# sara-nl/DDLBench

Hardware: AMD Instinct MI355X
Metric: images/sec (higher is better)
Workload: dtype bfloat16; 1 GPU; model=resnet50, global_batch=256, input=3x224x224, parallelism=dp1

## Files before the change

ddlbench_amd/ops/conv.py:

```python

from __future__ import annotations

import os

import torch
import torch.nn as nn
import torch.nn.functional as F

from ddlbench_amd import ops as _ops

_WGRAD = os.environ.get("DDLB_WGRAD", "mfma")

_CL = torch.channels_last


def _dw_to_weight_layout(dw32, weight):
    K, C, R, S = weight.shape
    return dw32.view(K, R, S, C).permute(0, 3, 1, 2).to(weight.dtype)


def _conv_backward(ctx, dy, add=None):
    ext = _ops.require_extension()
    x, weight = ctx.saved_tensors
    dy = dy.contiguous(memory_format=_CL)
    dx = dw = None
    if ctx.needs_input_grad[0]:
        w_perm = weight.permute(1, 2, 3, 0).contiguous()
        dx = ext.conv_igemm_dgrad(dy, w_perm, x.size(0), x.size(1),
                                  x.size(2), x.size(3), ctx.stride,
                                  ctx.pad, add)
    if ctx.needs_input_grad[1]:
        if _WGRAD == "mfma":
            dw = _dw_to_weight_layout(
                ext.conv_igemm_wgrad(x, dy, weight.shape[2],
                                     weight.shape[3], ctx.stride,
                                     ctx.pad), weight)
        else:
            dw = torch.ops.aten.convolution_backward(
                dy, x, weight, None, [ctx.stride, ctx.stride],
                [ctx.pad, ctx.pad], [1, 1], False, [0, 0], 1,
                [False, True, False])[1]
    return dx, dw


class _ConvMFMA(torch.autograd.Function):
    @staticmethod
    def forward(ctx, x, weight, stride, pad):
        ext = _ops.require_extension()
        x = x.contiguous(memory_format=_CL)
        w = weight.contiguous(memory_format=_CL)
        y = ext.conv_igemm_fwd(x, w, stride, pad)
        ctx.save_for_backward(x, weight)
        ctx.stride = stride
        ctx.pad = pad
        return y

    @staticmethod
    def backward(ctx, dy):
        dx, dw = _conv_backward(ctx, dy)
        return dx, dw, None, None


def conv2d_mfma(x, weight, stride=1, pad=0):
    return _ConvMFMA.apply(x, weight, stride, pad)


class _ConvMFMAJoin(torch.autograd.Function):

    @staticmethod
    def forward(ctx, x, weight, stride, pad):
        ext = _ops.require_extension()
        w = weight.contiguous(memory_format=_CL)
        y = ext.conv_igemm_fwd(x, w, stride, pad)
        ctx.save_for_backward(x, weight)
        ctx.stride = stride
        ctx.pad = pad
        ctx.set_materialize_grads(False)
        return y, x

    @staticmethod
    def backward(ctx, dy, dskip):
        if dy is None:
            return dskip, None, None, None
        if dskip is not None:
            dskip = dskip.contiguous(memory_format=_CL)
        dx, dw = _conv_backward(ctx, dy, dskip)
        return dx, dw, None, None


def join_enabled() -> bool:
    return os.environ.get("DDLB_JOIN", "1") != "0"


def mfma_eligible(conv: nn.Conv2d, x_dtype=torch.bfloat16) -> bool:
    return (x_dtype == torch.bfloat16
            and conv.groups == 1
            and conv.dilation == (1, 1)
            and conv.bias is None
            and conv.in_channels % 8 == 0
            and conv.out_channels % 8 == 0
            and conv.stride[0] == conv.stride[1]
            and conv.padding[0] == conv.padding[1]
            and conv.kernel_size[0] == conv.kernel_size[1])


class _NativeConv2d(nn.Module):

    tag = ""

    def __init__(self, conv: nn.Conv2d):
        super().__init__()
        self.in_channels = conv.in_channels
        self.out_channels = conv.out_channels
        self.kernel_size = conv.kernel_size
        self.stride = conv.stride[0]
        self.padding = conv.padding[0]
        self.weight = conv.weight

    def native(self, x):
        raise NotImplementedError

    def forward(self, x):
        if x.is_cuda and x.dtype == torch.bfloat16:
            return self.native(x)
        return F.conv2d(x, self.weight, None, self.stride, self.padding)

    def extra_repr(self):
        return (f"{self.in_channels}, {self.out_channels}, "
                f"k={self.kernel_size}, stride={self.stride}, "
                f"pad={self.padding} [{self.tag}]")


class Conv2dMFMA(_NativeConv2d):

    tag = "mfma"

    def native(self, x):
        return conv2d_mfma(x, self.weight, self.stride, self.padding)

    def forward_join(self, x):
        if (x.is_cuda and x.dtype == torch.bfloat16 and x.dim() == 4
                and x.is_contiguous(memory_format=_CL) and join_enabled()):
            return _ConvMFMAJoin.apply(x, self.weight, self.stride,
                                       self.padding)
        return self.forward(x), x


class _ConvStem(torch.autograd.Function):

    @staticmethod
    def forward(ctx, x, weight, stride, pad):
        ext = _ops.require_extension()
        x = x.contiguous(memory_format=_CL)
        w = weight.contiguous(memory_format=_CL)
        y = ext.conv_stem_fwd(x, w, stride, pad)
        ctx.save_for_backward(x, weight)
        ctx.stride = stride
        ctx.pad = pad
        return y

    @staticmethod
    def backward(ctx, dy):
        ext = _ops.require_extension()
        x, weight = ctx.saved_tensors
        dy = dy.contiguous(memory_format=_CL)
        dx = dw = None
        if ctx.needs_input_grad[0]:
            dx = torch.ops.aten.convolution_backward(
                dy, x, weight, None, [ctx.stride, ctx.stride],
                [ctx.pad, ctx.pad], [1, 1], False, [0, 0], 1,
                [True, False, False])[0]
        if ctx.needs_input_grad[1]:
            dw = _dw_to_weight_layout(
                ext.conv_stem_wgrad(x, dy, weight.shape[2], weight.shape[3],
                                    ctx.stride, ctx.pad), weight)
        return dx, dw, None, None


def conv2d_stem(x, weight, stride=1, pad=0):
    return _ConvStem.apply(x, weight, stride, pad)


def stem_eligible(conv: nn.Conv2d, x_dtype=torch.bfloat16) -> bool:
    return (x_dtype == torch.bfloat16
            and conv.groups == 1
            and conv.dilation == (1, 1)
            and conv.bias is None
            and 1 <= conv.in_channels <= 4
            and conv.out_channels % 8 == 0
            and 8 <= conv.out_channels <= 128
            and conv.kernel_size[0] == conv.kernel_size[1]
            and conv.kernel_size[0] in (3, 5, 7)
            and conv.stride[0] == conv.stride[1]
            and conv.stride[0] in (1, 2)
            and not isinstance(conv.padding, str)
            and conv.padding[0] == conv.padding[1]
            and 0 <= conv.padding[0] <= conv.kernel_size[0] // 2)


class Conv2dStem(_NativeConv2d):

    tag = "stem"

    def native(self, x):
        return conv2d_stem(x, self.weight, self.stride, self.padding)


def convert_convs(model: nn.Module, dtype=torch.bfloat16,
                  stem=None) -> int:
    if stem is None:
        stem = os.environ.get("DDLB_STEM", "library")
    if stem not in ("native", "library"):
        raise ValueError(f"stem must be 'native' or 'library', got {stem!r}")
    count = 0
    for parent in model.modules():
        for name, child in list(parent.named_children()):
            if not isinstance(child, nn.Conv2d):
                continue
            if mfma_eligible(child, dtype):
                setattr(parent, name, Conv2dMFMA(child))
                count += 1
            elif stem == "native" and stem_eligible(child, dtype):
                setattr(parent, name, Conv2dStem(child))
                count += 1
    if dtype == torch.bfloat16 and \
            os.environ.get("DDLB_MAXPOOL", "1") != "0":
        from ddlbench_amd.ops.pool import convert_maxpools
        count += convert_maxpools(model)
    return count
```

ddlbench_amd/ops/csrc/bindings.hip:

```cpp

#include <torch/extension.h>
#include <c10/hip/HIPStream.h>
#include <hip/hip_runtime.h>
#include <hip/hip_bf16.h>

#include <algorithm>
#include <stdexcept>
#include <unordered_map>
#include <vector>

#include "launchers.h"

using namespace ddlb;

namespace {

hipStream_t cur_stream() {
  return c10::hip::getCurrentHIPStream().stream();
}

void check_gpu_contig(const torch::Tensor& t, const char* name) {
  TORCH_CHECK(t.is_cuda(), name, " must be on the HIP device");
  TORCH_CHECK(t.is_contiguous(), name, " must be contiguous");
}

bool is_bf16(const torch::Tensor& t) {
  return t.scalar_type() == at::kBFloat16;
}

template <typename T>
T* dptr(const torch::Tensor& t) {
  return reinterpret_cast<T*>(t.data_ptr());
}

template <typename F>
auto dispatch_f32_bf16(bool bf16, F&& fn) {
  return bf16 ? fn(__hip_bfloat16{}) : fn(float{});
}
template <typename F>
auto dispatch_f32_bf16(const torch::Tensor& x, F&& fn) {
  return dispatch_f32_bf16(is_bf16(x), fn);
}

using WsCache = std::unordered_map<int, torch::Tensor>;
torch::Tensor cached_ws(WsCache& cache, const torch::Tensor& like,
                        at::ScalarType dtype, int64_t min_numel,
                        int64_t grow_floor = 0, bool zeroed = false) {
  torch::Tensor& t = cache[(int)like.get_device()];
  if (!t.defined() || t.numel() < min_numel) {
    const int64_t cap = std::max(min_numel, grow_floor);
    const auto opt = like.options().dtype(dtype);
    t = zeroed ? torch::zeros({cap}, opt) : torch::empty({cap}, opt);
  }
  return t;
}

torch::Tensor zero_page(const torch::Tensor& like) {
  static WsCache zp;
  return cached_ws(zp, like, at::kBFloat16, 16, 0, true);
}

torch::Tensor bn_sums_workspace(const torch::Tensor& like, int64_t C,
                                int64_t S) {
  static WsCache ws;
  return cached_ws(ws, like, at::kDouble, 2 * C * S, 1 << 18);
}

void check_conv_operand(const torch::Tensor& t, const char* name,
                        const char* op = "conv_igemm") {
  TORCH_CHECK(t.is_cuda() && t.scalar_type() == at::kBFloat16, op,
              ": bf16 HIP tensors only");
  TORCH_CHECK(t.is_contiguous(at::MemoryFormat::ChannelsLast), name,
              " must be channels_last");
}

int conv_out_size(int64_t H, int64_t pad, int64_t R, int64_t stride) {
  return (int)((H + 2 * pad - R) / stride + 1);
}

void check_conv_geometry(const char* op, int64_t N, int64_t H, int64_t W,
                         int64_t R, int64_t S, int64_t stride,
                         int64_t pad) {
  TORCH_CHECK(stride >= 1, op, ": stride must be >= 1");
  TORCH_CHECK(pad >= 0, op, ": pad must be >= 0");
  TORCH_CHECK(R >= 1 && S >= 1, op, ": kernel dims must be >= 1");
  TORCH_CHECK(N >= 1 && H >= 1 && W >= 1, op, ": empty input");
  TORCH_CHECK(H + 2 * pad >= R && W + 2 * pad >= S, op,
              ": kernel larger than the padded input");
}

void check_conv_dy(const char* op, const torch::Tensor& dy, int64_t N,
                   int64_t H, int64_t W, int64_t R, int64_t S,
                   int64_t stride, int64_t pad) {
  TORCH_CHECK(dy.size(0) == N, op, ": dy batch does not match x");
  TORCH_CHECK(dy.size(2) == conv_out_size(H, pad, R, stride) &&
                  dy.size(3) == conv_out_size(W, pad, S, stride),
              op, ": dy spatial dims do not match (H,W,R,S,stride,pad)");
}

torch::Tensor empty_nhwc(const torch::Tensor& like, int64_t N, int64_t C,
                         int64_t H, int64_t W) {
  return torch::empty({N, C, H, W}, like.options().memory_format(
                                        at::MemoryFormat::ChannelsLast));
}

}

void fused_sgd(torch::Tensor ptr_params, torch::Tensor ptr_grads,
               torch::Tensor ptr_moms, torch::Tensor prefix, int64_t total,
               double lr, double momentum, double weight_decay,
               bool first_step, bool bf16) {
  check_gpu_contig(ptr_params, "ptr_params");
  dispatch_f32_bf16(bf16, [&](auto tag) {
    launch_fused_sgd<decltype(tag)>(
        dptr<uintptr_t>(ptr_params), dptr<uintptr_t>(ptr_grads),
        dptr<uintptr_t>(ptr_moms), dptr<int64_t>(prefix),
        (int)ptr_params.numel(), total, (float)lr, (float)momentum,
        (float)weight_decay, first_step, cur_stream());
  });
}

void fused_adam(torch::Tensor ptr_params, torch::Tensor ptr_grads,
                torch::Tensor ptr_ms, torch::Tensor ptr_vs,
                torch::Tensor prefix, int64_t total, double lr,
                double beta1, double beta2, double eps,
                double weight_decay, double bc1, double bc2,
                bool decoupled_wd, bool bf16) {
  check_gpu_contig(ptr_params, "ptr_params");
  dispatch_f32_bf16(bf16, [&](auto tag) {
    launch_fused_adam<decltype(tag)>(
        dptr<uintptr_t>(ptr_params), dptr<uintptr_t>(ptr_grads),
        dptr<uintptr_t>(ptr_ms), dptr<uintptr_t>(ptr_vs),
        dptr<int64_t>(prefix), (int)ptr_params.numel(), total, (float)lr,
        (float)beta1, (float)beta2, (float)eps, (float)weight_decay,
        (float)bc1, (float)bc2, decoupled_wd, cur_stream());
  });
}

std::vector<torch::Tensor> bn_act_fwd(
    torch::Tensor x, c10::optional<torch::Tensor> res, torch::Tensor gamma,
    torch::Tensor beta, c10::optional<torch::Tensor> running_mean,
    c10::optional<torch::Tensor> running_var, bool training, double momentum,
    double eps, int64_t act, bool nhwc) {
  TORCH_CHECK(x.is_cuda(), "x must be on the HIP device");
  TORCH_CHECK(x.dim() == 4, "x must be 4-D");
  TORCH_CHECK(nhwc ? x.is_contiguous(at::MemoryFormat::ChannelsLast)
                   : x.is_contiguous(), "x layout mismatch");
  const int64_t N = x.size(0), C = x.size(1), HW = x.size(2) * x.size(3);
  auto s = cur_stream();
  auto fopt = x.options().dtype(at::kFloat);
  torch::Tensor mean = torch::empty({C}, fopt);
  torch::Tensor invstd = torch::empty({C}, fopt);
  if (training) {
    const int64_t S =
        bn_reduce_gridS(N, C, HW, nhwc, (int)x.element_size());
    torch::Tensor sums = bn_sums_workspace(x, C, S);
    dispatch_f32_bf16(x, [&](auto tag) {
      using T = decltype(tag);
      launch_bn_stats<T>(dptr<T>(x), dptr<double>(sums), N, C, HW, S, nhwc,
                         s);
    });
    launch_bn_finalize(
        dptr<double>(sums), dptr<float>(mean), dptr<float>(invstd),
        running_mean ? dptr<float>(*running_mean) : nullptr,
        running_var ? dptr<float>(*running_var) : nullptr, C, S,
        (double)(N * HW), (float)eps, (float)momentum, s);
  } else {
    TORCH_CHECK(running_mean && running_var,
                "eval mode needs running stats");
    mean.copy_(*running_mean);
    invstd.copy_((running_var->to(at::kFloat) + eps).rsqrt());
  }
  torch::Tensor y = torch::empty_like(x);
  const int64_t total = x.numel();
  torch::Tensor msk;
  const bool want_mask =
      training && act != 0 && nhwc && is_bf16(x) && C % 8 == 0;
  if (want_mask)
    msk = torch::empty({total / 8}, x.options().dtype(at::kByte));
  const bool mask_written = dispatch_f32_bf16(x, [&](auto tag) {
    using T = decltype(tag);
    return launch_bn_apply<T>(
        dptr<T>(x), res ? dptr<T>(*res) : nullptr, dptr<T>(y),
        dptr<float>(mean), dptr<float>(invstd), dptr<float>(gamma),
        dptr<float>(beta),
        want_mask ? msk.data_ptr<unsigned char>() : nullptr,
        C, HW, total, (int)act, nhwc, s);
  });
  if (mask_written) return {y, mean, invstd, msk};
  return {y, mean, invstd};
}

std::vector<torch::Tensor> bn_act_bwd(torch::Tensor dy,
                                      c10::optional<torch::Tensor> y_opt,
                                      torch::Tensor x, torch::Tensor mean,
                                      torch::Tensor invstd,
                                      torch::Tensor gamma, int64_t act,
                                      bool training, bool need_dres,
                                      bool nhwc,
                                      c10::optional<torch::Tensor> msk) {
  TORCH_CHECK(dy.is_cuda(), "dy must be on the HIP device");
  TORCH_CHECK(y_opt || msk,
              "bn_act_bwd needs y or the 1-bit activation mask");
  const int64_t N = x.size(0), C = x.size(1), HW = x.size(2) * x.size(3);
  auto s = cur_stream();
  auto fopt = x.options().dtype(at::kFloat);
  const int64_t S = bn_reduce_gridS(N, C, HW, nhwc, (int)x.element_size());
  torch::Tensor sums = bn_sums_workspace(x, C, S);
  torch::Tensor dgamma = torch::empty({C}, fopt);
  torch::Tensor dbeta = torch::empty({C}, fopt);
  torch::Tensor k = torch::empty({3, C}, fopt);
  torch::Tensor dx = torch::empty_like(x);
  torch::Tensor dres =
      need_dres ? torch::empty_like(x) : torch::Tensor();
  const int64_t total = x.numel();
  const unsigned char* mp =
      msk ? msk->data_ptr<unsigned char>() : nullptr;
  if (!is_bf16(x)) {
    TORCH_CHECK(y_opt, "fp32 backward needs y");
    mp = nullptr;
  }
  dispatch_f32_bf16(x, [&](auto tag) {
    using T = decltype(tag);
    const T* yp = y_opt ? dptr<T>(*y_opt) : nullptr;
    launch_bn_bwd_reduce<T>(dptr<T>(dy), yp, dptr<T>(x), dptr<float>(mean),
                            dptr<float>(invstd), dptr<double>(sums), mp, N,
                            C, HW, S, (int)act, nhwc, s);
    launch_bn_bwd_finalize(dptr<double>(sums), dptr<float>(gamma),
                           dptr<float>(invstd), dptr<float>(dgamma),
                           dptr<float>(dbeta), dptr<float>(k), C, S,
                           (double)(N * HW), training, s);
    launch_bn_bwd_dx<T>(dptr<T>(dy), yp, dptr<T>(x), dptr<float>(mean),
                        dptr<float>(invstd), dptr<float>(k), dptr<T>(dx),
                        need_dres ? dptr<T>(dres) : nullptr, mp, C, HW,
                        total, (int)act, nhwc, s);
  });
  if (need_dres) return {dx, dgamma, dbeta, dres};
  return {dx, dgamma, dbeta};
}

std::vector<torch::Tensor> ce_fwd(torch::Tensor logits,
                                  torch::Tensor target) {
  check_gpu_contig(logits, "logits");
  const int64_t B = logits.size(0), K = logits.size(1);
  auto s = cur_stream();
  auto fopt = logits.options().dtype(at::kFloat);
  torch::Tensor lse = torch::empty({B}, fopt);
  torch::Tensor loss_sum = torch::zeros({1}, fopt);
  dispatch_f32_bf16(logits, [&](auto tag) {
    using T = decltype(tag);
    launch_ce_fwd<T>(dptr<T>(logits), dptr<int64_t>(target),
                     dptr<float>(lse), dptr<float>(loss_sum), B, K, s);
  });
  return {loss_sum, lse};
}

torch::Tensor ce_bwd(torch::Tensor logits, torch::Tensor target,
                     torch::Tensor lse, torch::Tensor gscale) {
  const int64_t B = logits.size(0), K = logits.size(1);
  auto s = cur_stream();
  torch::Tensor dx = torch::empty_like(logits);
  dispatch_f32_bf16(logits, [&](auto tag) {
    using T = decltype(tag);
    launch_ce_bwd<T>(dptr<T>(logits), dptr<int64_t>(target),
                     dptr<float>(lse), dptr<float>(gscale), dptr<T>(dx), B,
                     K, s);
  });
  return dx;
}

torch::Tensor conv_igemm_fwd(torch::Tensor x, torch::Tensor w,
                             int64_t stride, int64_t pad) {
  TORCH_CHECK(x.dim() == 4 && w.dim() == 4, "conv_igemm: 4-D tensors only");
  check_conv_operand(x, "x", "conv_igemm");
  check_conv_operand(w, "w", "conv_igemm");
  TORCH_CHECK(w.device() == x.device(), "conv_igemm: w must be on x's device");
  const int N = x.size(0), C = x.size(1), H = x.size(2), W = x.size(3);
  const int K = w.size(0), R = w.size(2), S = w.size(3);
  TORCH_CHECK(w.size(1) == C, "conv_igemm: weight C does not match x");
  TORCH_CHECK(C % 8 == 0, "conv_igemm fwd needs C % 8 == 0");
  TORCH_CHECK(K >= 1, "conv_igemm: empty weight");
  check_conv_geometry("conv_igemm", N, H, W, R, S, stride, pad);
  const int OH = conv_out_size(H, pad, R, stride);
  const int OW = conv_out_size(W, pad, S, stride);
  auto y = empty_nhwc(x, N, K, OH, OW);
  launch_conv_igemm(x.data_ptr(), w.data_ptr(), y.data_ptr(),
                    zero_page(x).data_ptr(), N, H, W, C, K, OH, OW, R, S,
                    (int)stride, (int)pad, 0, nullptr,
                    cur_stream());
  return y;
}

torch::Tensor conv_igemm_dgrad(torch::Tensor dy, torch::Tensor w_perm,
                               int64_t N, int64_t C, int64_t H, int64_t W,
                               int64_t stride, int64_t pad,
                               c10::optional<torch::Tensor> add) {
  TORCH_CHECK(dy.dim() == 4 && w_perm.dim() == 4,
              "conv_igemm: 4-D tensors only");
  check_conv_operand(dy, "dy", "conv_igemm");
  TORCH_CHECK(w_perm.is_cuda() && w_perm.scalar_type() == at::kBFloat16 &&
                  w_perm.device() == dy.device(),
              "conv_igemm: w_perm must be a bf16 tensor on dy's device");
  TORCH_CHECK(w_perm.is_contiguous(), "w_perm must be contiguous");
  if (add) {
    check_conv_operand(*add, "add", "conv_igemm");
    TORCH_CHECK(add->dim() == 4 && add->size(0) == N &&
                    add->size(1) == C && add->size(2) == H &&
                    add->size(3) == W,
                "add must have dx's shape (N,C,H,W)");
    TORCH_CHECK(add->device() == dy.device(),
                "add must be on dy's device");
  }
  const int K = dy.size(1), OH = dy.size(2), OW = dy.size(3);
  const int R = w_perm.size(1), S = w_perm.size(2);
  TORCH_CHECK(K % 8 == 0, "conv_igemm dgrad needs K % 8 == 0");
  TORCH_CHECK(C >= 1 && w_perm.size(0) == C && w_perm.size(3) == K,
              "conv_igemm: w_perm must be (C,R,S,K) for dx's C and dy's K");
  check_conv_geometry("conv_igemm", N, H, W, R, S, stride, pad);
  check_conv_dy("conv_igemm", dy, N, H, W, R, S, stride, pad);
  auto dx = empty_nhwc(dy, N, C, H, W);
  const bool sparse = stride == 2 && (R == 1 || S == 1);
  if (sparse) dx.zero_();
  launch_conv_igemm(dy.data_ptr(), w_perm.data_ptr(), dx.data_ptr(),
                    zero_page(dy).data_ptr(), (int)N, (int)H, (int)W,
                    (int)C, K, OH, OW, R, S, (int)stride, (int)pad,
                    1, add && !sparse ? add->data_ptr() : nullptr,
                    cur_stream());
  if (add && sparse) dx.add_(*add);
  return dx;
}

torch::Tensor conv_igemm_wgrad(torch::Tensor x, torch::Tensor dy,
                               int64_t R, int64_t S, int64_t stride,
                               int64_t pad) {
  TORCH_CHECK(x.dim() == 4 && dy.dim() == 4, "conv_wgrad: 4-D tensors only");
  check_conv_operand(x, "x", "conv_wgrad");
  check_conv_operand(dy, "dy", "conv_wgrad");
  TORCH_CHECK(dy.device() == x.device(),
              "conv_wgrad: dy must be on x's device");
  const int N = x.size(0), C = x.size(1), H = x.size(2), W = x.size(3);
  const int K = dy.size(1), OH = dy.size(2), OW = dy.size(3);
  TORCH_CHECK(C % 8 == 0 && K % 8 == 0,
              "conv_wgrad needs C %% 8 == 0 and K %% 8 == 0");
  TORCH_CHECK(K >= 1, "conv_wgrad: empty dy");
  check_conv_geometry("conv_wgrad", N, H, W, R, S, stride, pad);
  check_conv_dy("conv_wgrad", dy, N, H, W, R, S, stride, pad);
  auto dw = torch::empty({K, R * S * C},
                         x.options().dtype(at::kFloat));
  static WsCache wgws;
  auto part = cached_ws(wgws, x, at::kFloat, kConvWgradPartCap);
  launch_conv_wgrad(x.data_ptr(), dy.data_ptr(), dw.data_ptr<float>(),
                    part.data_ptr<float>(), (long)part.numel(),
                    zero_page(x).data_ptr(), N, H, W, C, K, OH, OW, (int)R,
                    (int)S, (int)stride, (int)pad, cur_stream());
  return dw;
}

py::list conv_igemm_plan_py(int64_t N, int64_t C, int64_t H, int64_t W,
                            int64_t K, int64_t R, int64_t S, int64_t stride,
                            int64_t pad, bool dgrad) {
  check_conv_geometry("conv_igemm_plan", N, H, W, R, S, stride, pad);
  const ConvIgemmPlan plan = conv_igemm_plan(
      (int)N, (int)H, (int)W, (int)C, (int)K,
      conv_out_size(H, pad, R, stride), conv_out_size(W, pad, S, stride),
      (int)R, (int)S, (int)stride, (int)pad, dgrad ? 1 : 0);
  py::list out;
  for (int i = 0; i < plan.n; ++i) {
    const ConvIgemmLaunch& e = plan.e[i];
    py::dict d;
    d["structure"] = e.v2 ? "v2" : "v1";
    d["mode"] = e.mode;
    d["BM"] = e.bm;
    d["BN"] = e.bn;
    d["LIN"] = e.lin != 0;
    d["M"] = e.M;
    d["Nd"] = e.Nd;
    d["Kd"] = e.Kd;
    d["cls"] = py::make_tuple(e.cls_a, e.cls_b);
    d["taps"] = py::make_tuple(e.nr, e.ns);
    out.append(d);
  }
  return out;
}

py::dict conv_wgrad_plan_py(int64_t N, int64_t C, int64_t H, int64_t W,
                            int64_t K, int64_t R, int64_t S, int64_t stride,
                            int64_t pad) {
  check_conv_geometry("conv_wgrad_plan", N, H, W, R, S, stride, pad);
  const ConvWgradPlan pl = conv_wgrad_plan(
      (int)N, (int)C, (int)K, conv_out_size(H, pad, R, stride),
      conv_out_size(W, pad, S, stride), (int)R, (int)S, (int)stride,
      (int)pad, kConvWgradPartCap);
  py::dict d;
  d["TK"] = pl.tk;
  d["TR"] = pl.tr;
  d["ring"] = pl.ring;
  d["r1"] = pl.r1 != 0;
  d["split"] = pl.split;
  d["p_per"] = pl.p_per;
  d["steps"] = pl.steps;
  d["tail"] = pl.tail;
  d["psb"] = pl.psb;
  return d;
}

static void check_stem_shape(int64_t C, int64_t K, int64_t R, int64_t S,
                             int64_t stride, int64_t pad) {
  TORCH_CHECK(C >= 1 && C <= 4, "conv_stem needs 1 <= C <= 4");
  TORCH_CHECK(R == S && (R == 3 || R == 5 || R == 7),
              "conv_stem needs a square 3x3, 5x5 or 7x7 kernel");
  TORCH_CHECK(stride == 1 || stride == 2, "conv_stem needs stride 1 or 2");
  TORCH_CHECK(pad >= 0 && pad <= R / 2, "conv_stem needs 0 <= pad <= R/2");
  TORCH_CHECK(K % 8 == 0 && K >= 8 && K <= 128,
              "conv_stem needs K % 8 == 0 and K <= 128");
}

torch::Tensor conv_stem_fwd(torch::Tensor x, torch::Tensor w,
                            int64_t stride, int64_t pad) {
  TORCH_CHECK(x.dim() == 4 && w.dim() == 4, "conv_stem: 4-D tensors only");
  check_conv_operand(x, "x", "conv_stem");
  check_conv_operand(w, "w", "conv_stem");
  const int N = x.size(0), C = x.size(1), H = x.size(2), W = x.size(3);
  const int K = w.size(0), R = w.size(2), S = w.size(3);
  TORCH_CHECK(w.size(1) == C, "conv_stem: weight C mismatch");
  check_stem_shape(C, K, R, S, stride, pad);
  const int OH = conv_out_size(H, pad, R, stride);
  const int OW = conv_out_size(W, pad, S, stride);
  TORCH_CHECK(N >= 1 && H + 2 * pad >= R && W + 2 * pad >= S,
              "conv_stem: empty output");
  auto y = empty_nhwc(x, N, K, OH, OW);
  launch_conv_stem_fwd(x.data_ptr(), w.data_ptr(), y.data_ptr(), N, H, W, C,
                       K, OH, OW, R, (int)stride, (int)pad, cur_stream());
  return y;
}

torch::Tensor conv_stem_wgrad(torch::Tensor x, torch::Tensor dy, int64_t R,
                              int64_t S, int64_t stride, int64_t pad) {
  TORCH_CHECK(x.dim() == 4 && dy.dim() == 4, "conv_stem: 4-D tensors only");
  check_conv_operand(x, "x", "conv_stem");
  check_conv_operand(dy, "dy", "conv_stem");
  const int N = x.size(0), C = x.size(1), H = x.size(2), W = x.size(3);
  const int K = dy.size(1), OH = dy.size(2), OW = dy.size(3);
  check_stem_shape(C, K, R, S, stride, pad);
  TORCH_CHECK(N >= 1 && dy.size(0) == N && OH >= 1 && OW >= 1 &&
                  OH == conv_out_size(H, pad, R, stride) &&
                  OW == conv_out_size(W, pad, S, stride),
              "conv_stem: dy shape does not match x");
  const int64_t total = (int64_t)K * R * S * C;
  auto dw = torch::empty({K, R * S * C}, x.options().dtype(at::kFloat));
  static WsCache stws;
  auto part = cached_ws(stws, x, at::kFloat,
                        total * conv_stem_wgrad_chunks(N, OH, OW, K));
  launch_conv_stem_wgrad(x.data_ptr(), dy.data_ptr(), dw.data_ptr<float>(),
                         part.data_ptr<float>(), N, H, W, C, K, OH, OW,
                         (int)R, (int)stride, (int)pad, cur_stream());
  return dw;
}

std::vector<torch::Tensor> maxpool_fwd(torch::Tensor x, int64_t k,
                                       int64_t stride, int64_t pad) {
  TORCH_CHECK(x.is_cuda() && x.scalar_type() == at::kBFloat16,
              "maxpool: bf16 HIP tensors only");
  TORCH_CHECK(x.is_contiguous(at::MemoryFormat::ChannelsLast),
              "maxpool: x must be channels_last");
  const int64_t N = x.size(0), C = x.size(1);
  const int H = (int)x.size(2), W = (int)x.size(3);
  TORCH_CHECK(C % 8 == 0, "maxpool needs C %% 8 == 0");
  const int OH = (H + 2 * (int)pad - (int)k) / (int)stride + 1;
  const int OW = (W + 2 * (int)pad - (int)k) / (int)stride + 1;
  auto y = torch::empty({N, C, OH, OW},
                        x.options().memory_format(
                            at::MemoryFormat::ChannelsLast));
  auto idx = torch::empty({N * OH * OW * C},
                          x.options().dtype(at::kByte));
  launch_maxpool_fwd(x.data_ptr(), y.data_ptr(),
                     idx.data_ptr<unsigned char>(), N, C, H, W, OH, OW,
                     (int)k, (int)stride, (int)pad, cur_stream());
  return {y, idx};
}

torch::Tensor maxpool_bwd(torch::Tensor dy, torch::Tensor idx,
                          int64_t H, int64_t W, int64_t k,
                          int64_t stride, int64_t pad) {
  TORCH_CHECK(dy.is_cuda() && dy.scalar_type() == at::kBFloat16,
              "maxpool: bf16 HIP tensors only");
  TORCH_CHECK(dy.is_contiguous(at::MemoryFormat::ChannelsLast),
              "maxpool: dy must be channels_last");
  const int64_t N = dy.size(0), C = dy.size(1);
  const int OH = (int)dy.size(2), OW = (int)dy.size(3);
  auto dx = torch::empty({N, C, H, W},
                         dy.options().memory_format(
                             at::MemoryFormat::ChannelsLast));
  launch_maxpool_bwd(dy.data_ptr(), idx.data_ptr<unsigned char>(),
                     dx.data_ptr(), N, C, (int)H, (int)W, OH, OW,
                     (int)k, (int)stride, (int)pad, cur_stream());
  return dx;
}

torch::Tensor dw3x3_fwd(torch::Tensor x, torch::Tensor w, int64_t stride,
                        bool nhwc) {
  TORCH_CHECK(x.is_cuda(), "x must be on the HIP device");
  check_gpu_contig(w, "w");
  const int64_t N = x.size(0), C = x.size(1), H = x.size(2), W = x.size(3);
  const int64_t OH = (H + 2 - 3) / stride + 1, OW = (W + 2 - 3) / stride + 1;
  auto s = cur_stream();
  torch::Tensor y = nhwc
      ? torch::empty({N, C, OH, OW}, x.options().memory_format(
            at::MemoryFormat::ChannelsLast))
      : torch::empty({N, C, OH, OW}, x.options());
  dispatch_f32_bf16(x, [&](auto tag) {
    using T = decltype(tag);
    launch_dw3x3_fwd<T>(dptr<T>(x), dptr<float>(w), dptr<T>(y), N, C, H, W,
                        OH, OW, (int)stride, nhwc, s);
  });
  return y;
}

std::vector<torch::Tensor> dw3x3_bwd(torch::Tensor x, torch::Tensor w,
                                     torch::Tensor dy, int64_t stride,
                                     bool need_dx, bool need_dw,
                                     bool nhwc) {
  const int64_t N = x.size(0), C = x.size(1), H = x.size(2), W = x.size(3);
  const int64_t OH = dy.size(2), OW = dy.size(3);
  auto s = cur_stream();
  torch::Tensor dx, dwt;
  if (need_dx) {
    dx = torch::empty_like(x);
    dispatch_f32_bf16(x, [&](auto tag) {
      using T = decltype(tag);
      launch_dw3x3_bwd_dx<T>(dptr<T>(dy), dptr<float>(w), dptr<T>(dx), N, C,
                             H, W, OH, OW, (int)stride, nhwc, s);
    });
  }
  if (need_dw) {
    torch::Tensor acc = torch::zeros({C * 9}, x.options().dtype(at::kDouble));
    dispatch_f32_bf16(x, [&](auto tag) {
      using T = decltype(tag);
      launch_dw3x3_bwd_dw<T>(dptr<T>(x), dptr<T>(dy), dptr<double>(acc), N,
                             C, H, W, OH, OW, (int)stride, nhwc, s);
    });
    dwt = acc.to(at::kFloat).view({C, 1, 3, 3});
  }
  return {dx, dwt};
}

torch::Tensor revert_varlen(torch::Tensor x, torch::Tensor lengths) {
  check_gpu_contig(x, "x");
  TORCH_CHECK(x.dim() == 3, "x must be (T, B, F)");
  TORCH_CHECK(lengths.scalar_type() == at::kLong, "lengths must be int64");
  const int64_t T = x.size(0), B = x.size(1), F = x.size(2);
  auto out = torch::empty_like(x);
  auto s = cur_stream();
  dispatch_f32_bf16(x, [&](auto tag) {
    using E = decltype(tag);
    launch_revert_varlen<E>(dptr<E>(x), dptr<E>(out),
                            dptr<int64_t>(lengths), T, B, F, s);
  });
  return out;
}

torch::Tensor varlen_mask(torch::Tensor lengths, int64_t T) {
  TORCH_CHECK(lengths.is_cuda(), "lengths must be on the HIP device");
  const int64_t B = lengths.size(0);
  auto mask = torch::empty({T, B}, lengths.options().dtype(at::kByte));
  launch_varlen_mask(dptr<int64_t>(lengths), dptr<uint8_t>(mask), T, B,
                     cur_stream());
  return mask;
}

PYBIND11_MODULE(TORCH_EXTENSION_NAME, m) {
  m.doc() = "ddlbench_amd gfx950 HIP kernels";
  m.def("fused_sgd", &fused_sgd, "fused multi-tensor SGD step");
  m.def("fused_adam", &fused_adam, "fused multi-tensor Adam/AdamW step");
  m.def("bn_act_fwd", &bn_act_fwd, "fused BN+act(+res) forward");
  m.def("set_bn_variant", &set_bn_variant,
        "BN kernel variant for A/B probes (0 auto, 1 scalar-group, 2 vec)");
  m.def("bn_act_bwd", &bn_act_bwd, "fused BN+act(+res) backward");
  m.def("maxpool_fwd", &maxpool_fwd, "NHWC bf16 max-pool forward");
  m.def("maxpool_bwd", &maxpool_bwd, "NHWC bf16 max-pool backward");
  m.def("conv_igemm_fwd", &conv_igemm_fwd,
        "NHWC bf16 MFMA implicit-GEMM conv forward");
  m.def("conv_igemm_dgrad", &conv_igemm_dgrad,
        "NHWC bf16 MFMA implicit-GEMM conv data-grad (+ optional addend)",
        py::arg("dy"), py::arg("w_perm"), py::arg("N"), py::arg("C"),
        py::arg("H"), py::arg("W"), py::arg("stride"), py::arg("pad"),
        py::arg("add") = py::none());
  m.def("conv_igemm_wgrad", &conv_igemm_wgrad,
        "NHWC bf16 MFMA implicit-GEMM conv weight-grad (fp32 out)");
  m.def("conv_igemm_plan", &conv_igemm_plan_py,
        "launches conv_igemm_fwd/dgrad make for a shape (host only)",
        py::arg("N"), py::arg("C"), py::arg("H"), py::arg("W"),
        py::arg("K"), py::arg("R"), py::arg("S"), py::arg("stride"),
        py::arg("pad"), py::arg("dgrad"));
  m.def("conv_wgrad_plan", &conv_wgrad_plan_py,
        "tile/split/steps conv_igemm_wgrad uses for a shape (host only)",
        py::arg("N"), py::arg("C"), py::arg("H"), py::arg("W"),
        py::arg("K"), py::arg("R"), py::arg("S"), py::arg("stride"),
        py::arg("pad"));
  m.def("conv_stem_fwd", &conv_stem_fwd,
        "NHWC bf16 MFMA stem conv (C < 8) forward");
  m.def("conv_stem_wgrad", &conv_stem_wgrad,
        "NHWC bf16 MFMA stem conv (C < 8) weight-grad (fp32 out)");
  m.def("ce_fwd", &ce_fwd, "cross-entropy forward");
  m.def("ce_bwd", &ce_bwd, "cross-entropy backward");
  m.def("revert_varlen", &revert_varlen,
        "reverse each batch element's valid time prefix (T,B,F)");
  m.def("varlen_mask", &varlen_mask, "valid-timestep mask (T,B) uint8");
  m.def("dw3x3_fwd", &dw3x3_fwd, "depthwise 3x3 forward");
  m.def("dw3x3_bwd", &dw3x3_bwd, "depthwise 3x3 backward");
}
```

ddlbench_amd/ops/csrc/bn_act.hip:

```cpp

#include "common.h"
#include "launchers.h"
#include <stdint.h>
#include <stdexcept>
#include <string>

namespace {

template <int ACT> DEV float act_fwd(float v) {
  if (ACT == 1) return fmaxf(v, 0.f);
  if (ACT == 2) return fminf(fmaxf(v, 0.f), 6.f);
  return v;
}

template <int ACT> DEV float act_mask(float y) {
  if (ACT == 1) return y > 0.f ? 1.f : 0.f;
  if (ACT == 2) return (y > 0.f && y < 6.f) ? 1.f : 0.f;
  return 1.f;
}

}

int g_bn_variant = 0;
void ddlb::set_bn_variant(int v) { g_bn_variant = v; }

template <typename T>
__global__ void bn_stats_kernel(const T* __restrict__ x, double* __restrict__ sums,
                                int64_t N, int64_t C, int64_t HW) {
  __shared__ double tmp[8];
  const int64_t c = blockIdx.x;
  const int64_t total = N * HW;
  const int64_t per = (total + gridDim.y - 1) / gridDim.y;
  const int64_t begin = (int64_t)blockIdx.y * per;
  const int64_t end = i64min(begin + per, total);
  double s = 0.0, ss = 0.0;
  for (int64_t i = begin + threadIdx.x; i < end; i += blockDim.x) {
    const int64_t n = i / HW, r = i - n * HW;
    const float v = to_f32(x[(n * C + c) * HW + r]);
    s += v;
    ss += fma((double)v, (double)v, 0.0);
  }
  auto op = [](double v) { return wave_reduce_sum(v); };
  s = block_reduce(s, tmp, op, 0.0);
  __syncthreads();
  ss = block_reduce(ss, tmp, op, 0.0);
  if (threadIdx.x == 0) {
    sums[((int64_t)blockIdx.y * 2 + 0) * C + c] = s;
    sums[((int64_t)blockIdx.y * 2 + 1) * C + c] = ss;
  }
}

template <typename T>
__global__ void bn_stats_nhwc_kernel(const T* __restrict__ x,
                                     double* __restrict__ sums,
                                     int64_t rows, int64_t C, int CG) {
  __shared__ double tmp[2 * 256];
  const int ci = threadIdx.x % CG;
  const int rj = threadIdx.x / CG;
  const int RG = blockDim.x / CG;
  const int64_t c = (int64_t)blockIdx.x * CG + ci;
  const bool active = (c < C) && (rj < RG);
  const int64_t per = (rows + gridDim.y - 1) / gridDim.y;
  const int64_t begin = (int64_t)blockIdx.y * per;
  const int64_t end = i64min(begin + per, rows);
  double s = 0.0, ss = 0.0;
  if (active) {
    int64_t r = begin + rj;
    const int64_t step = RG;
    for (; r + 3 * step < end; r += 4 * step) {
      float v0 = to_f32(x[(r + 0 * step) * C + c]);
      float v1 = to_f32(x[(r + 1 * step) * C + c]);
      float v2 = to_f32(x[(r + 2 * step) * C + c]);
      float v3 = to_f32(x[(r + 3 * step) * C + c]);
      s += (double)v0 + v1 + v2 + v3;
      ss += fma((double)v0, v0, fma((double)v1, v1,
                fma((double)v2, v2, (double)v3 * v3)));
    }
    for (; r < end; r += step) {
      const float v = to_f32(x[r * C + c]);
      s += v;
      ss += fma((double)v, (double)v, 0.0);
    }
  }
  tmp[threadIdx.x] = s;
  tmp[256 + threadIdx.x] = ss;
  __syncthreads();
  if (rj == 0 && c < C) {
    for (int j = 1; j < RG; ++j) {
      s += tmp[j * CG + ci];
      ss += tmp[256 + j * CG + ci];
    }
    sums[((int64_t)blockIdx.y * 2 + 0) * C + c] = s;
    sums[((int64_t)blockIdx.y * 2 + 1) * C + c] = ss;
  }
}

template <typename T>
__global__ void bn_stats_nhwc_vec_kernel(const T* __restrict__ x,
                                         double* __restrict__ sums,
                                         int64_t rows, int64_t C, int CG8) {
  typedef __attribute__((ext_vector_type(8))) short short8x;
  __shared__ float tmp[2][256][8];
  const int ci = threadIdx.x % CG8;
  const int rj = threadIdx.x / CG8;
  const int RG = blockDim.x / CG8;
  const int64_t c0 = ((int64_t)blockIdx.x * CG8 + ci) * 8;
  const bool active = (c0 < C) && (rj < RG);
  const int64_t per = (rows + gridDim.y - 1) / gridDim.y;
  const int64_t begin = (int64_t)blockIdx.y * per;
  const int64_t end = i64min(begin + per, rows);
  float s[8] = {0, 0, 0, 0, 0, 0, 0, 0};
  float ss[8] = {0, 0, 0, 0, 0, 0, 0, 0};
  if (active) {
    const short8x* xv = reinterpret_cast<const short8x*>(x);
    for (int64_t r = begin + rj; r < end; r += RG) {
      short8x v = xv[(r * C + c0) / 8];
#pragma unroll
      for (int j = 0; j < 8; ++j) {
        __hip_bfloat16 h;
        unsigned short u = (unsigned short)v[j];
        __builtin_memcpy(&h, &u, 2);
        const float f = __bfloat162float(h);
        s[j] += f;
        ss[j] = fmaf(f, f, ss[j]);
      }
    }
  }
#pragma unroll
  for (int j = 0; j < 8; ++j) {
    tmp[0][threadIdx.x][j] = s[j];
    tmp[1][threadIdx.x][j] = ss[j];
  }
  __syncthreads();
  if (rj == 0 && c0 < C) {
    for (int g = 1; g < RG; ++g)
#pragma unroll
      for (int j = 0; j < 8; ++j) {
        s[j] += tmp[0][g * CG8 + ci][j];
        ss[j] += tmp[1][g * CG8 + ci][j];
      }
#pragma unroll
    for (int j = 0; j < 8; ++j) {
      sums[((int64_t)blockIdx.y * 2 + 0) * C + c0 + j] = (double)s[j];
      sums[((int64_t)blockIdx.y * 2 + 1) * C + c0 + j] = (double)ss[j];
    }
  }
}

__global__ void bn_stats_nhwc_vec_f32_kernel(const float* __restrict__ x,
                                             double* __restrict__ sums,
                                             int64_t rows, int64_t C,
                                             int CG4) {
  typedef __attribute__((ext_vector_type(4))) float float4x;
  __shared__ float tmp[2][256][4];
  const int ci = threadIdx.x % CG4;
  const int rj = threadIdx.x / CG4;
  const int RG = blockDim.x / CG4;
  const int64_t c0 = ((int64_t)blockIdx.x * CG4 + ci) * 4;
  const bool active = (c0 < C) && (rj < RG);
  const int64_t per = (rows + gridDim.y - 1) / gridDim.y;
  const int64_t begin = (int64_t)blockIdx.y * per;
  const int64_t end = i64min(begin + per, rows);
  float s[4] = {0, 0, 0, 0}, ss[4] = {0, 0, 0, 0};
  if (active) {
    const float4x* xv = reinterpret_cast<const float4x*>(x);
    for (int64_t r = begin + rj; r < end; r += RG) {
      float4x v = xv[(r * C + c0) / 4];
#pragma unroll
      for (int j = 0; j < 4; ++j) {
        s[j] += v[j];
        ss[j] = fmaf(v[j], v[j], ss[j]);
      }
    }
  }
#pragma unroll
  for (int j = 0; j < 4; ++j) {
    tmp[0][threadIdx.x][j] = s[j];
    tmp[1][threadIdx.x][j] = ss[j];
  }
  __syncthreads();
  if (rj == 0 && c0 < C) {
    for (int g = 1; g < RG; ++g)
#pragma unroll
      for (int j = 0; j < 4; ++j) {
        s[j] += tmp[0][g * CG4 + ci][j];
        ss[j] += tmp[1][g * CG4 + ci][j];
      }
#pragma unroll
    for (int j = 0; j < 4; ++j) {
      sums[((int64_t)blockIdx.y * 2 + 0) * C + c0 + j] = (double)s[j];
      sums[((int64_t)blockIdx.y * 2 + 1) * C + c0 + j] = (double)ss[j];
    }
  }
}

__global__ void bn_finalize_kernel(const double* __restrict__ sums,
                                   float* __restrict__ mean,
                                   float* __restrict__ invstd,
                                   float* __restrict__ running_mean,
                                   float* __restrict__ running_var,
                                   int64_t C, int64_t S, double count,
                                   float eps, float momentum) {
  __shared__ double tmp[16];
  const int64_t c = blockIdx.x;
  double s = 0.0, ss = 0.0;
  for (int64_t b = threadIdx.x; b < S; b += blockDim.x) {
    s += sums[(b * 2 + 0) * C + c];
    ss += sums[(b * 2 + 1) * C + c];
  }
  auto op = [](double v) { return wave_reduce_sum(v); };
  s = block_reduce(s, tmp, op, 0.0);
  __syncthreads();
  ss = block_reduce(ss, tmp, op, 0.0);
  if (threadIdx.x != 0) return;
  const double m = s / count;
  double var = ss / count - m * m;
  var = var < 0.0 ? 0.0 : var;
  mean[c] = (float)m;
  invstd[c] = (float)rsqrt(var + (double)eps);
  if (running_mean != nullptr) {
    const double unbiased = count > 1.0 ? var * count / (count - 1.0) : var;
    running_mean[c] = (1.f - momentum) * running_mean[c] + momentum * (float)m;
    running_var[c] = (1.f - momentum) * running_var[c] + momentum * (float)unbiased;
  }
}

template <typename T, int ACT, bool ADD>
__global__ void bn_apply_kernel(const T* __restrict__ x,
                                const T* __restrict__ res,
                                T* __restrict__ y,
                                const float* __restrict__ mean,
                                const float* __restrict__ invstd,
                                const float* __restrict__ gamma,
                                const float* __restrict__ beta,
                                int64_t C, int64_t cdiv, int64_t total) {
  const int64_t stride = (int64_t)gridDim.x * blockDim.x;
  for (int64_t i = (int64_t)blockIdx.x * blockDim.x + threadIdx.x; i < total;
       i += stride) {
    const int64_t c = (i / cdiv) % C;
    float v = (to_f32(x[i]) - mean[c]) * invstd[c] * gamma[c] + beta[c];
    if (ADD) v += to_f32(res[i]);
    y[i] = from_f32<T>(act_fwd<ACT>(v));
  }
}

typedef __attribute__((ext_vector_type(8))) short short8v;
typedef __attribute__((ext_vector_type(4))) float float4v;

template <typename T> struct vec8;
template <> struct vec8<float> {
  using type = __attribute__((ext_vector_type(8))) float;
};
template <> struct vec8<__hip_bfloat16> { using type = short8v; };

DEV float elt_f32(const short8v& v, int j) {
  __hip_bfloat16 h;
  unsigned short u = (unsigned short)v[j];
  __builtin_memcpy(&h, &u, 2);
  return __bfloat162float(h);
}
DEV float elt_f32(const __attribute__((ext_vector_type(8))) float& v,
                  int j) { return v[j]; }

template <typename T>
DEV void set_elt(short8v& v, int j, float f) {
  __hip_bfloat16 h = __float2bfloat16(f);
  unsigned short u;
  __builtin_memcpy(&u, &h, 2);
  v[j] = (short)u;
}
template <typename T>
DEV void set_elt(__attribute__((ext_vector_type(8))) float& v, int j,
                 float f) { v[j] = f; }

template <typename T, int ACT, bool ADD, bool NHWC>
__global__ void bn_apply_vec_kernel(const T* __restrict__ x,
                                    const T* __restrict__ res,
                                    T* __restrict__ y,
                                    const float* __restrict__ mean,
                                    const float* __restrict__ invstd,
                                    const float* __restrict__ gamma,
                                    const float* __restrict__ beta,
                                    int64_t C, int64_t cdiv,
                                    int64_t total8) {
  using V = typename vec8<T>::type;
  const V* xv = reinterpret_cast<const V*>(x);
  const V* rv = reinterpret_cast<const V*>(res);
  V* yv = reinterpret_cast<V*>(y);
  const int64_t stride = (int64_t)gridDim.x * blockDim.x;
  for (int64_t i = (int64_t)blockIdx.x * blockDim.x + threadIdx.x;
       i < total8; i += stride) {
    const int64_t e0 = i * 8;
    V vx = xv[i];
    V vr;
    if (ADD) vr = rv[i];
    V vy;
    if (NHWC) {
      const int64_t c0 = e0 % C;
#pragma unroll
      for (int j = 0; j < 8; ++j) {
        const int64_t c = c0 + j;
        float v = (elt_f32(vx, j) - mean[c]) * invstd[c] * gamma[c]
                  + beta[c];
        if (ADD) v += elt_f32(vr, j);
        set_elt<T>(vy, j, act_fwd<ACT>(v));
      }
    } else {
      const int64_t c = (e0 / cdiv) % C;
      const float mu = mean[c], is = invstd[c], g = gamma[c], b = beta[c];
#pragma unroll
      for (int j = 0; j < 8; ++j) {
        float v = (elt_f32(vx, j) - mu) * is * g + b;
        if (ADD) v += elt_f32(vr, j);
        set_elt<T>(vy, j, act_fwd<ACT>(v));
      }
    }
    yv[i] = vy;
  }
}

template <typename T, int ACT, bool ADD, bool NHWC>
__global__ void bn_bwd_dx_vec_kernel(const T* __restrict__ dy,
                                     const T* __restrict__ y,
                                     const T* __restrict__ x,
                                     const float* __restrict__ mean,
                                     const float* __restrict__ invstd,
                                     const float* __restrict__ k,
                                     T* __restrict__ dx,
                                     T* __restrict__ dres, int64_t C,
                                     int64_t cdiv, int64_t total8) {
  using V = typename vec8<T>::type;
  const V* dyv = reinterpret_cast<const V*>(dy);
  const V* yv = reinterpret_cast<const V*>(y);
  const V* xv = reinterpret_cast<const V*>(x);
  V* dxv = reinterpret_cast<V*>(dx);
  V* drv = reinterpret_cast<V*>(dres);
  const int64_t stride = (int64_t)gridDim.x * blockDim.x;
  for (int64_t i = (int64_t)blockIdx.x * blockDim.x + threadIdx.x;
       i < total8; i += stride) {
    const int64_t e0 = i * 8;
    V vdy = dyv[i], vy = yv[i], vx = xv[i];
    V vdx, vdr;
#pragma unroll
    for (int j = 0; j < 8; ++j) {
      const int64_t c = NHWC ? (e0 % C + j) : ((e0 / cdiv) % C);
      const float g = elt_f32(vdy, j) * act_mask<ACT>(elt_f32(vy, j));
      const float xhat = (elt_f32(vx, j) - mean[c]) * invstd[c];
      set_elt<T>(vdx, j, k[c] * (g - k[C + c] - xhat * k[2 * C + c]));
      if (ADD) set_elt<T>(vdr, j, g);
    }
    dxv[i] = vdx;
    if (ADD) drv[i] = vdr;
  }
}

template <typename T, int ACT, bool ADD>
__global__ void bn_apply_nhwc_kernel2(const T* __restrict__ x,
                                      const T* __restrict__ res,
                                      T* __restrict__ y,
                                      const float* __restrict__ mean,
                                      const float* __restrict__ invstd,
                                      const float* __restrict__ gamma,
                                      const float* __restrict__ beta,
                                      unsigned char* __restrict__ msk,
                                      int64_t rows, int64_t C, int CG8) {
  typedef __attribute__((ext_vector_type(8))) short short8x;
  const int ci = threadIdx.x % CG8;
  const int rj = threadIdx.x / CG8;
  const int RG = blockDim.x / CG8;
  const int64_t c0 = ((int64_t)blockIdx.x * CG8 + ci) * 8;
  if (c0 >= C || rj >= RG) return;
  float sc[8], sh[8];
#pragma unroll
  for (int j = 0; j < 8; ++j) {
    sc[j] = invstd[c0 + j] * gamma[c0 + j];
    sh[j] = beta[c0 + j] - mean[c0 + j] * sc[j];
  }
  const int64_t per = (rows + gridDim.y - 1) / gridDim.y;
  const int64_t begin = (int64_t)blockIdx.y * per;
  const int64_t end = i64min(begin + per, rows);
  const short8x* xv = reinterpret_cast<const short8x*>(x);
  const short8x* rv = reinterpret_cast<const short8x*>(res);
  short8x* yv = reinterpret_cast<short8x*>(y);
  for (int64_t r = begin + rj; r < end; r += RG) {
    const int64_t i8 = (r * C + c0) / 8;
    short8x vx = xv[i8];
    short8x vr;
    if (ADD) vr = rv[i8];
    short8x vy;
    unsigned mbits = 0;
#pragma unroll
    for (int j = 0; j < 8; ++j) {
      __hip_bfloat16 h;
      unsigned short u = (unsigned short)vx[j];
      __builtin_memcpy(&h, &u, 2);
      float v = fmaf(__bfloat162float(h), sc[j], sh[j]);
      if (ADD) {
        u = (unsigned short)vr[j];
        __builtin_memcpy(&h, &u, 2);
        v += __bfloat162float(h);
      }
      if (ACT != 0 && act_mask<ACT>(v) > 0.f) mbits |= 1u << j;
      h = __float2bfloat16(act_fwd<ACT>(v));
      __builtin_memcpy(&u, &h, 2);
      vy[j] = (short)u;
    }
    yv[i8] = vy;
    if (ACT != 0 && msk != nullptr) msk[i8] = (unsigned char)mbits;
  }
}

template <typename T, int ACT, bool ADD, bool MASKED = false>
__global__ void bn_bwd_dx_nhwc_kernel2(const T* __restrict__ dy,
                                       const T* __restrict__ y,
                                       const T* __restrict__ x,
                                       const float* __restrict__ mean,
                                       const float* __restrict__ invstd,
                                       const float* __restrict__ k,
                                       T* __restrict__ dx,
                                       T* __restrict__ dres,
                                       const unsigned char* __restrict__ msk,
                                       int64_t rows,
                                       int64_t C, int CG8) {
  typedef __attribute__((ext_vector_type(8))) short short8x;
  const int ci = threadIdx.x % CG8;
  const int rj = threadIdx.x / CG8;
  const int RG = blockDim.x / CG8;
  const int64_t c0 = ((int64_t)blockIdx.x * CG8 + ci) * 8;
  if (c0 >= C || rj >= RG) return;
  float k1[8], k2[8], k3[8], mu[8], is[8];
#pragma unroll
  for (int j = 0; j < 8; ++j) {
    k1[j] = k[c0 + j];
    k2[j] = k[C + c0 + j];
    k3[j] = k[2 * C + c0 + j];
    mu[j] = mean[c0 + j];
    is[j] = invstd[c0 + j];
  }
  const int64_t per = (rows + gridDim.y - 1) / gridDim.y;
  const int64_t begin = (int64_t)blockIdx.y * per;
  const int64_t end = i64min(begin + per, rows);
  const short8x* dyv = reinterpret_cast<const short8x*>(dy);
  const short8x* yv = reinterpret_cast<const short8x*>(y);
  const short8x* xv = reinterpret_cast<const short8x*>(x);
  short8x* dxv = reinterpret_cast<short8x*>(dx);
  short8x* drv = reinterpret_cast<short8x*>(dres);
  for (int64_t r = begin + rj; r < end; r += RG) {
    const int64_t i8 = (r * C + c0) / 8;
    short8x vdy = dyv[i8], vx = xv[i8];
    short8x vy;
    unsigned mb = 0;
    if (MASKED) mb = msk[i8];
    else vy = yv[i8];
    short8x vdx, vdr;
#pragma unroll
    for (int j = 0; j < 8; ++j) {
      __hip_bfloat16 h;
      unsigned short u;
      u = (unsigned short)vdy[j];
      __builtin_memcpy(&h, &u, 2);
      const float fdy = __bfloat162float(h);
      float gate;
      if (MASKED) {
        gate = (float)((mb >> j) & 1u);
      } else {
        u = (unsigned short)vy[j];
        __builtin_memcpy(&h, &u, 2);
        gate = act_mask<ACT>(__bfloat162float(h));
      }
      u = (unsigned short)vx[j];
      __builtin_memcpy(&h, &u, 2);
      const float fx = __bfloat162float(h);
      const float g = fdy * gate;
      const float xhat = (fx - mu[j]) * is[j];
      h = __float2bfloat16(k1[j] * (g - k2[j] - xhat * k3[j]));
      __builtin_memcpy(&u, &h, 2);
      vdx[j] = (short)u;
      if (ADD) {
        h = __float2bfloat16(g);
        __builtin_memcpy(&u, &h, 2);
        vdr[j] = (short)u;
      }
    }
    dxv[i8] = vdx;
    if (ADD) drv[i8] = vdr;
  }
}

template <typename T, int ACT>
__global__ void bn_bwd_reduce_kernel(const T* __restrict__ dy,
                                     const T* __restrict__ y,
                                     const T* __restrict__ x,
                                     const float* __restrict__ mean,
                                     const float* __restrict__ invstd,
                                     double* __restrict__ sums,
                                     int64_t N, int64_t C, int64_t HW) {
  __shared__ double tmp[8];
  const int64_t c = blockIdx.x;
  const float mu = mean[c], is = invstd[c];
  const int64_t total = N * HW;
  const int64_t per = (total + gridDim.y - 1) / gridDim.y;
  const int64_t begin = (int64_t)blockIdx.y * per;
  const int64_t end = i64min(begin + per, total);
  double sdy = 0.0, sdyx = 0.0;
  for (int64_t i = begin + threadIdx.x; i < end; i += blockDim.x) {
    const int64_t n = i / HW, r = i - n * HW;
    const int64_t idx = (n * C + c) * HW + r;
    const float g = to_f32(dy[idx]) * act_mask<ACT>(to_f32(y[idx]));
    const float xhat = (to_f32(x[idx]) - mu) * is;
    sdy += g;
    sdyx += fma((double)g, (double)xhat, 0.0);
  }
  auto op = [](double v) { return wave_reduce_sum(v); };
  sdy = block_reduce(sdy, tmp, op, 0.0);
  __syncthreads();
  sdyx = block_reduce(sdyx, tmp, op, 0.0);
  if (threadIdx.x == 0) {
    sums[((int64_t)blockIdx.y * 2 + 0) * C + c] = sdy;
    sums[((int64_t)blockIdx.y * 2 + 1) * C + c] = sdyx;
  }
}

template <typename T, int ACT, bool MASKED = false>
__global__ void bn_bwd_reduce_nhwc_kernel(const T* __restrict__ dy,
                                          const T* __restrict__ y,
                                          const T* __restrict__ x,
                                          const float* __restrict__ mean,
                                          const float* __restrict__ invstd,
                                          double* __restrict__ sums,
                                          const unsigned char* __restrict__
                                              msk,
                                          int64_t rows, int64_t C, int CG) {
  __shared__ double tmp[2 * 256];
  const int ci = threadIdx.x % CG;
  const int rj = threadIdx.x / CG;
  const int RG = blockDim.x / CG;
  const int64_t c = (int64_t)blockIdx.x * CG + ci;
  const bool active = (c < C) && (rj < RG);
  const int64_t per = (rows + gridDim.y - 1) / gridDim.y;
  const int64_t begin = (int64_t)blockIdx.y * per;
  const int64_t end = i64min(begin + per, rows);
  double sdy = 0.0, sdyx = 0.0;
  if (active) {
    const float mu = mean[c], is = invstd[c];
    const int cbit = (int)(c & 7);
    for (int64_t r = begin + rj; r < end; r += RG) {
      const int64_t idx = r * C + c;
      float gate;
      if (MASKED)
        gate = (float)((msk[idx >> 3] >> cbit) & 1u);
      else
        gate = act_mask<ACT>(to_f32(y[idx]));
      const float g = to_f32(dy[idx]) * gate;
      const float xhat = (to_f32(x[idx]) - mu) * is;
      sdy += g;
      sdyx += fma((double)g, (double)xhat, 0.0);
    }
  }
  tmp[threadIdx.x] = sdy;
  tmp[256 + threadIdx.x] = sdyx;
  __syncthreads();
  if (rj == 0 && c < C) {
    for (int j = 1; j < RG; ++j) {
      sdy += tmp[j * CG + ci];
      sdyx += tmp[256 + j * CG + ci];
    }
    sums[((int64_t)blockIdx.y * 2 + 0) * C + c] = sdy;
    sums[((int64_t)blockIdx.y * 2 + 1) * C + c] = sdyx;
  }
}

template <typename T, int ACT, bool MASKED = false>
__global__ void bn_bwd_reduce_nhwc_vec_kernel(
    const T* __restrict__ dy, const T* __restrict__ y,
    const T* __restrict__ x, const float* __restrict__ mean,
    const float* __restrict__ invstd, double* __restrict__ sums,
    const unsigned char* __restrict__ msk,
    int64_t rows, int64_t C, int CG8) {
  typedef __attribute__((ext_vector_type(8))) short short8x;
  __shared__ float tmp[2][256][8];
  const int ci = threadIdx.x % CG8;
  const int rj = threadIdx.x / CG8;
  const int RG = blockDim.x / CG8;
  const int64_t c0 = ((int64_t)blockIdx.x * CG8 + ci) * 8;
  const bool active = (c0 < C) && (rj < RG);
  const int64_t per = (rows + gridDim.y - 1) / gridDim.y;
  const int64_t begin = (int64_t)blockIdx.y * per;
  const int64_t end = i64min(begin + per, rows);
  float sdy[8] = {0, 0, 0, 0, 0, 0, 0, 0};
  float sdyx[8] = {0, 0, 0, 0, 0, 0, 0, 0};
  float mu[8], is[8];
  if (active) {
#pragma unroll
    for (int j = 0; j < 8; ++j) {
      mu[j] = mean[c0 + j];
      is[j] = invstd[c0 + j];
    }
    const short8x* dyv = reinterpret_cast<const short8x*>(dy);
    const short8x* yv = reinterpret_cast<const short8x*>(y);
    const short8x* xv = reinterpret_cast<const short8x*>(x);
    for (int64_t r = begin + rj; r < end; r += RG) {
      const int64_t i8 = (r * C + c0) / 8;
      short8x vdy = dyv[i8], vx = xv[i8];
      short8x vy;
      unsigned mb = 0;
      if (MASKED) mb = msk[i8];
      else vy = yv[i8];
#pragma unroll
      for (int j = 0; j < 8; ++j) {
        __hip_bfloat16 h;
        unsigned short u;
        u = (unsigned short)vdy[j];
        __builtin_memcpy(&h, &u, 2);
        const float fdy = __bfloat162float(h);
        float gate;
        if (MASKED) {
          gate = (float)((mb >> j) & 1u);
        } else {
          u = (unsigned short)vy[j];
          __builtin_memcpy(&h, &u, 2);
          gate = act_mask<ACT>(__bfloat162float(h));
        }
        u = (unsigned short)vx[j];
        __builtin_memcpy(&h, &u, 2);
        const float fx = __bfloat162float(h);
        const float g = fdy * gate;
        sdy[j] += g;
        sdyx[j] = fmaf(g, (fx - mu[j]) * is[j], sdyx[j]);
      }
    }
  }
#pragma unroll
  for (int j = 0; j < 8; ++j) {
    tmp[0][threadIdx.x][j] = sdy[j];
    tmp[1][threadIdx.x][j] = sdyx[j];
  }
  __syncthreads();
  if (rj == 0 && c0 < C) {
    for (int g = 1; g < RG; ++g)
#pragma unroll
      for (int j = 0; j < 8; ++j) {
        sdy[j] += tmp[0][g * CG8 + ci][j];
        sdyx[j] += tmp[1][g * CG8 + ci][j];
      }
#pragma unroll
    for (int j = 0; j < 8; ++j) {
      sums[((int64_t)blockIdx.y * 2 + 0) * C + c0 + j] = (double)sdy[j];
      sums[((int64_t)blockIdx.y * 2 + 1) * C + c0 + j] = (double)sdyx[j];
    }
  }
}

__global__ void bn_bwd_finalize_kernel(const double* __restrict__ sums,
                                       const float* __restrict__ gamma,
                                       const float* __restrict__ invstd,
                                       float* __restrict__ dgamma,
                                       float* __restrict__ dbeta,
                                       float* __restrict__ k,
                                       int64_t C, int64_t S, double count,
                                       int training) {
  __shared__ double tmp[16];
  const int64_t c = blockIdx.x;
  double sdy = 0.0, sdyx = 0.0;
  for (int64_t b = threadIdx.x; b < S; b += blockDim.x) {
    sdy += sums[(b * 2 + 0) * C + c];
    sdyx += sums[(b * 2 + 1) * C + c];
  }
  auto op = [](double v) { return wave_reduce_sum(v); };
  sdy = block_reduce(sdy, tmp, op, 0.0);
  __syncthreads();
  sdyx = block_reduce(sdyx, tmp, op, 0.0);
  if (threadIdx.x != 0) return;
  dgamma[c] = (float)sdyx;
  dbeta[c] = (float)sdy;
  k[c] = gamma[c] * invstd[c];
  k[C + c] = training ? (float)(sdy / count) : 0.f;
  k[2 * C + c] = training ? (float)(sdyx / count) : 0.f;
}

template <typename T, int ACT, bool ADD>
__global__ void bn_bwd_dx_kernel(const T* __restrict__ dy,
                                 const T* __restrict__ y,
                                 const T* __restrict__ x,
                                 const float* __restrict__ mean,
                                 const float* __restrict__ invstd,
                                 const float* __restrict__ k,
                                 T* __restrict__ dx, T* __restrict__ dres,
                                 int64_t C, int64_t cdiv, int64_t total) {
  const int64_t stride = (int64_t)gridDim.x * blockDim.x;
  for (int64_t i = (int64_t)blockIdx.x * blockDim.x + threadIdx.x; i < total;
       i += stride) {
    const int64_t c = (i / cdiv) % C;
    const float g = to_f32(dy[i]) * act_mask<ACT>(to_f32(y[i]));
    const float xhat = (to_f32(x[i]) - mean[c]) * invstd[c];
    dx[i] = from_f32<T>(k[c] * (g - k[C + c] - xhat * k[2 * C + c]));
    if (ADD) dres[i] = from_f32<T>(g);
  }
}

static inline int elementwise_grid(int64_t total, int block) {
  int64_t want = (total + block - 1) / block;
  return (int)i64min(want > 0 ? want : 1, 256 * 8);
}


struct BnGeom { bool vec; int64_t cblocks, S; };

static BnGeom bn_reduce_geom(int64_t rows, int64_t C, int elsize) {
  BnGeom g;
  const bool vec_ok = (elsize == 2 && C % 8 == 0) ||
                      (elsize == 4 && C % 4 == 0);
  g.vec = vec_ok && (g_bn_variant == 2 ||
                     (g_bn_variant == 0 && C <= 512 && elsize == 2));
  if (g.vec) {
    const int64_t lanes = elsize == 2 ? C / 8 : C / 4;
    const int64_t CG = i64min(lanes, 64);
    g.cblocks = (lanes + CG - 1) / CG;
  } else {
    const int64_t CG = C >= 64 ? 64 : C;
    g.cblocks = (C + CG - 1) / CG;
  }
  g.S = i64min(i64max(rows / 16, 1), i64max(2048 / g.cblocks, 1));
  return g;
}

int64_t ddlb::bn_reduce_gridS(int64_t N, int64_t C, int64_t HW, int nhwc,
                              int elsize) {
  if (nhwc) return bn_reduce_geom(N * HW, C, elsize).S;
  int64_t S = i64min((N * HW + 255) / 256, i64max(2048 / C, 1));
  return i64max(S, 1);
}

template <typename T>
void ddlb::launch_bn_stats(const T* x, double* sums, int64_t N, int64_t C,
                           int64_t HW, int64_t S, int nhwc,
                           hipStream_t stream) {
  const int block = 256;
  if (nhwc) {
    const int64_t rows = N * HW;
    const BnGeom g = bn_reduce_geom(rows, C, (int)sizeof(T));
    if (g.vec && sizeof(T) == 2) {
      const int CG8 = (int)i64min(C / 8, 64);
      hipLaunchKernelGGL((bn_stats_nhwc_vec_kernel<T>),
                         dim3(g.cblocks, S),
                         dim3(block), 0, stream, x, sums, rows, C, CG8);
    } else if (g.vec && sizeof(T) == 4) {
      const int CG4 = (int)i64min(C / 4, 64);
      hipLaunchKernelGGL(bn_stats_nhwc_vec_f32_kernel, dim3(g.cblocks, S),
                         dim3(block), 0, stream, (const float*)x, sums,
                         rows, C, CG4);
    } else {
      const int CG = C >= 64 ? 64 : (int)C;
      hipLaunchKernelGGL((bn_stats_nhwc_kernel<T>), dim3(g.cblocks, S),
                         dim3(block), 0, stream, x, sums, rows, C, CG);
    }
  } else {
    hipLaunchKernelGGL((bn_stats_kernel<T>), dim3(C, S), dim3(block), 0,
                       stream, x, sums, N, C, HW);
  }
  HIP_CHECK_LAST();
}

void ddlb::launch_bn_finalize(double* sums, float* mean, float* invstd,
                              float* rm, float* rv, int64_t C, int64_t S,
                              double count, float eps, float momentum,
                              hipStream_t stream) {
  const int block = 1024;
  hipLaunchKernelGGL(bn_finalize_kernel, dim3((unsigned)C),
                     dim3(block), 0, stream, sums, mean, invstd, rm, rv, C,
                     S, count, eps, momentum);
  HIP_CHECK_LAST();
}

template <typename T>
bool ddlb::launch_bn_apply(const T* x, const T* res, T* y, const float* mean,
                           const float* invstd, const float* gamma,
                           const float* beta, unsigned char* msk, int64_t C,
                           int64_t HW, int64_t total, int act, int nhwc,
                           hipStream_t stream) {
  const int block = 256;
  const int64_t cdiv = nhwc ? 1 : HW;
  const bool vec8ok = (total % 8 == 0) &&
                      (nhwc ? (C % 8 == 0) : (HW % 8 == 0));
  const int64_t rows_nhwc = nhwc ? total / C : 0;
  if (nhwc && sizeof(T) == 2 && C % 8 == 0 && g_bn_variant != 1 &&
      (rows_nhwc >= 32768 || (msk != nullptr && act != 0) ||
       g_bn_variant == 2)) {
    const int64_t rows = total / C;
    const int CG8 = (int)i64min(C / 8, 64);
    const int64_t cblocks = (C / 8 + CG8 - 1) / CG8;
    int64_t S = i64min(i64max(rows / 16, 1), i64max(2048 / cblocks, 1));
    const bool add = res != nullptr;
#define KCASE(ACT, ADD)                                                     \
    hipLaunchKernelGGL((bn_apply_nhwc_kernel2<T, ACT, ADD>),                \
                       dim3(cblocks, S), dim3(block), 0, stream, x, res,    \
                       y, mean, invstd, gamma, beta, msk, rows, C, CG8)
    if (act == 0) { if (add) KCASE(0, true); else KCASE(0, false); }
    else if (act == 1) { if (add) KCASE(1, true); else KCASE(1, false); }
    else { if (add) KCASE(2, true); else KCASE(2, false); }
#undef KCASE
    HIP_CHECK_LAST();
    return act != 0 && msk != nullptr;
  }
  if (vec8ok) {
    const int64_t total8 = total / 8;
    const int grid8 = elementwise_grid(total8, block);
    const bool add = res != nullptr;
#define VCASE(ACT, ADD, NHWC)                                               \
    hipLaunchKernelGGL((bn_apply_vec_kernel<T, ACT, ADD, NHWC>),            \
                       dim3(grid8), dim3(block), 0, stream, x, res, y,      \
                       mean, invstd, gamma, beta, C, cdiv, total8)
#define VSEL(ACT)                                                           \
    do { if (nhwc) { if (add) VCASE(ACT, true, true);                       \
                     else VCASE(ACT, false, true); }                        \
         else { if (add) VCASE(ACT, true, false);                           \
                else VCASE(ACT, false, false); } } while (0)
    if (act == 0) VSEL(0);
    else if (act == 1) VSEL(1);
    else VSEL(2);
#undef VSEL
#undef VCASE
    HIP_CHECK_LAST();
    return false;
  }
  const int grid = elementwise_grid(total, block);
#define CASE(ACT, ADD)                                                       \
  hipLaunchKernelGGL((bn_apply_kernel<T, ACT, ADD>), dim3(grid), dim3(block), \
                     0, stream, x, res, y, mean, invstd, gamma, beta, C,    \
                     cdiv, total)
  const bool add = res != nullptr;
  if (act == 0 && !add) CASE(0, false);
  else if (act == 0 && add) CASE(0, true);
  else if (act == 1 && !add) CASE(1, false);
  else if (act == 1 && add) CASE(1, true);
  else if (act == 2 && !add) CASE(2, false);
  else CASE(2, true);
#undef CASE
  HIP_CHECK_LAST();
  return false;
}

template <typename T>
void ddlb::launch_bn_bwd_reduce(const T* dy, const T* y, const T* x,
                                const float* mean, const float* invstd,
                                double* sums, const unsigned char* msk,
                                int64_t N, int64_t C, int64_t HW, int64_t S,
                                int act, int nhwc, hipStream_t stream) {
  const int block = 256;
  if (nhwc) {
    const int64_t rows = N * HW;
    const bool masked = msk != nullptr && act != 0;
    const BnGeom g = bn_reduce_geom(rows, C, (int)sizeof(T));
    if (g.vec && sizeof(T) == 2) {
      const int CG8 = (int)i64min(C / 8, 64);
#define CASE(ACT, MSK)                                                      \
      hipLaunchKernelGGL((bn_bwd_reduce_nhwc_vec_kernel<T, ACT, MSK>),      \
                         dim3(g.cblocks, S), dim3(block), 0, stream, dy,    \
                         y, x, mean, invstd, sums, msk, rows, C, CG8)
      if (act == 0) CASE(0, false);
      else if (act == 1) { if (masked) CASE(1, true); else CASE(1, false); }
      else { if (masked) CASE(2, true); else CASE(2, false); }
#undef CASE
    } else {
      const int CG = C >= 64 ? 64 : (int)C;
#define CASE(ACT, MSK)                                                      \
      hipLaunchKernelGGL((bn_bwd_reduce_nhwc_kernel<T, ACT, MSK>),          \
                         dim3(g.cblocks, S), dim3(block), 0, stream, dy,    \
                         y, x, mean, invstd, sums, msk, rows, C, CG)
      if (act == 0) CASE(0, false);
      else if (act == 1) { if (masked) CASE(1, true); else CASE(1, false); }
      else { if (masked) CASE(2, true); else CASE(2, false); }
#undef CASE
    }
  } else {
#define CASE(ACT)                                                          \
    hipLaunchKernelGGL((bn_bwd_reduce_kernel<T, ACT>), dim3(C, S),         \
                       dim3(block), 0, stream, dy, y, x, mean, invstd,     \
                       sums, N, C, HW)
    if (act == 0) CASE(0);
    else if (act == 1) CASE(1);
    else CASE(2);
#undef CASE
  }
  HIP_CHECK_LAST();
}

void ddlb::launch_bn_bwd_finalize(double* sums, const float* gamma,
                                  const float* invstd, float* dgamma,
                                  float* dbeta, float* k, int64_t C, int64_t S,
                                  double count, int training,
                                  hipStream_t stream) {
  const int block = 1024;
  hipLaunchKernelGGL(bn_bwd_finalize_kernel, dim3((unsigned)C),
                     dim3(block), 0, stream, sums, gamma, invstd, dgamma,
                     dbeta, k, C, S, count, training);
  HIP_CHECK_LAST();
}

template <typename T>
void ddlb::launch_bn_bwd_dx(const T* dy, const T* y, const T* x,
                            const float* mean, const float* invstd,
                            const float* k, T* dx, T* dres,
                            const unsigned char* msk, int64_t C, int64_t HW,
                            int64_t total, int act, int nhwc,
                            hipStream_t stream) {
  const int block = 256;
  const int64_t cdiv = nhwc ? 1 : HW;
  const bool vec8ok = (total % 8 == 0) &&
                      (nhwc ? (C % 8 == 0) : (HW % 8 == 0));
  const int64_t rows_nhwc = nhwc ? total / C : 0;
  if (nhwc && sizeof(T) == 2 && C % 8 == 0 &&
      ((g_bn_variant != 1 && rows_nhwc >= 32768) || msk != nullptr ||
       g_bn_variant == 2)) {
    const int64_t rows = total / C;
    const int CG8 = (int)i64min(C / 8, 64);
    const int64_t cblocks = (C / 8 + CG8 - 1) / CG8;
    int64_t S = i64min(i64max(rows / 16, 1), i64max(2048 / cblocks, 1));
    const bool add = dres != nullptr;
    const bool masked = msk != nullptr && act != 0;
#define KCASE(ACT, ADD, MSK)                                                \
    hipLaunchKernelGGL((bn_bwd_dx_nhwc_kernel2<T, ACT, ADD, MSK>),          \
                       dim3(cblocks, S), dim3(block), 0, stream, dy, y, x,  \
                       mean, invstd, k, dx, dres, msk, rows, C, CG8)
#define KSEL(ACT)                                                           \
    do { if (add) { if (masked) KCASE(ACT, true, true);                     \
                    else KCASE(ACT, true, false); }                         \
         else { if (masked) KCASE(ACT, false, true);                        \
                else KCASE(ACT, false, false); } } while (0)
    if (act == 0) KSEL(0);
    else if (act == 1) KSEL(1);
    else KSEL(2);
#undef KSEL
#undef KCASE
    HIP_CHECK_LAST();
    return;
  }
  if (vec8ok) {
    const int64_t total8 = total / 8;
    const int grid8 = elementwise_grid(total8, block);
    const bool add = dres != nullptr;
#define VCASE(ACT, ADD, NHWC)                                               \
    hipLaunchKernelGGL((bn_bwd_dx_vec_kernel<T, ACT, ADD, NHWC>),           \
                       dim3(grid8), dim3(block), 0, stream, dy, y, x,       \
                       mean, invstd, k, dx, dres, C, cdiv, total8)
#define VSEL(ACT)                                                           \
    do { if (nhwc) { if (add) VCASE(ACT, true, true);                       \
                     else VCASE(ACT, false, true); }                        \
         else { if (add) VCASE(ACT, true, false);                           \
                else VCASE(ACT, false, false); } } while (0)
    if (act == 0) VSEL(0);
    else if (act == 1) VSEL(1);
    else VSEL(2);
#undef VSEL
#undef VCASE
    HIP_CHECK_LAST();
    return;
  }
  const int grid = elementwise_grid(total, block);
#define CASE(ACT, ADD)                                                    \
  hipLaunchKernelGGL((bn_bwd_dx_kernel<T, ACT, ADD>), dim3(grid),         \
                     dim3(block), 0, stream, dy, y, x, mean, invstd, k,   \
                     dx, dres, C, cdiv, total)
  const bool add = dres != nullptr;
  if (act == 0 && !add) CASE(0, false);
  else if (act == 0 && add) CASE(0, true);
  else if (act == 1 && !add) CASE(1, false);
  else if (act == 1 && add) CASE(1, true);
  else if (act == 2 && !add) CASE(2, false);
  else CASE(2, true);
#undef CASE
  HIP_CHECK_LAST();
}

#define INSTANTIATE(T)                                                        \
  template void ddlb::launch_bn_stats<T>(                                     \
      const T*, double*, int64_t, int64_t, int64_t, int64_t, int,             \
      hipStream_t);                                                           \
  template bool ddlb::launch_bn_apply<T>(                                     \
      const T*, const T*, T*, const float*, const float*, const float*,       \
      const float*, unsigned char*, int64_t, int64_t, int64_t, int, int,      \
      hipStream_t);                                                           \
  template void ddlb::launch_bn_bwd_reduce<T>(                                \
      const T*, const T*, const T*, const float*, const float*, double*,      \
      const unsigned char*, int64_t, int64_t, int64_t, int64_t, int, int,     \
      hipStream_t);                                                           \
  template void ddlb::launch_bn_bwd_dx<T>(                                    \
      const T*, const T*, const T*, const float*, const float*, const float*, \
      T*, T*, const unsigned char*, int64_t, int64_t, int64_t, int, int,      \
      hipStream_t);

INSTANTIATE(float)
INSTANTIATE(__hip_bfloat16)
#undef INSTANTIATE
```

ddlbench_amd/ops/csrc/conv_wgrad.hip:

```cpp

#include "mfma_common.h"
#include "launchers.h"
#include <stdint.h>
#include <stdexcept>
#include <string>

using bf16 = __hip_bfloat16;
typedef __attribute__((address_space(3))) const short* lds_cptr;

#define WG_BKP 64

struct WgradParams {
  const bf16* x;
  const bf16* dy;
  float* dw;
  float* part;
  const bf16* zero;
  int N, H, W, C, K, OH, OW, R, S, stride, pad;
  long P;
  long RSC;
  int split_p;
};

namespace {

DEV void wg_decode_chunk(int d, int& p, int& ch) {
  const int g = d >> 7;
  const int r = d & 127;
  const int phalf = r >> 6;
  const int r2 = r & 63;
  p = (r2 >> 3) * 8 + phalf * 4 + ((r2 >> 1) & 3);
  ch = g * 16 + (r2 & 1) * 8;
}

DEV bf16x8 wg_tr_frag(const short* img, int group, int ks, int lane) {
  bf16x4 lo, hi;
  lds_cptr base = (lds_cptr)(img + group * (WG_BKP * 16) + ks * 4 * 64 +
                             lane * 4);
  asm volatile("ds_read_b64_tr_b16 %0, %2\n\t"
               "ds_read_b64_tr_b16 %1, %2 offset:%3"
               : "=&v"(lo), "=&v"(hi)
               : "v"(base), "i"(WG_BKP * 8 * 2));
  bf16x8 f;
#pragma unroll
  for (int e = 0; e < 4; ++e) {
    f[e] = lo[e];
    f[4 + e] = hi[e];
  }
  return f;
}

template <int TKt, int TRt, int WR, int WC, int TPB, bool R1, bool RING2>
__global__ __launch_bounds__(TPB, RING2 ? 4 : 2)
void conv_wgrad2_kernel(WgradParams q) {
  constexpr int NBUF = RING2 ? 2 : 3;
  constexpr int GA = TKt * 8 / TPB;
  constexpr int GB = TRt * 8 / TPB;
  constexpr int MFS = TKt / WR / 16;
  constexpr int NFS = TRt / WC / 16;
  static_assert(WR * WC == TPB / 64, "wave count");
  static_assert(GA >= 1 && GB >= 1, "tile vs threads");
  extern __shared__ __attribute__((aligned(16))) char smem[];
  short* lds = reinterpret_cast<short*>(smem);
  auto aimg = [&](int buf) { return lds + buf * WG_BKP * (TKt + TRt); };
  auto bimg = [&](int buf) { return aimg(buf) + WG_BKP * TKt; };

  const int tid = threadIdx.x;
  const int lane = tid & 63;
  const int wid = tid >> 6;

  const int nk = (q.K + TKt - 1) / TKt;
  const int nr = (int)((q.RSC + TRt - 1) / TRt);
  const long block = blockIdx.x;
  const long kb = (block % nk) * TKt;
  const long rb = ((block / nk) % nr) * TRt;
  const int ps_idx = (int)(block / ((long)nk * nr));
  const long p_per = (q.P + q.split_p - 1) / q.split_p;
  const long p_begin = ps_idx * p_per;
  const long p_end = i64min(p_begin + p_per, q.P);
  const int nsteps = (int)((p_end - p_begin + WG_BKP - 1) / WG_BKP);

  int a_p[GA], a_ch[GA];
  const bf16* a_src[GA];
  bool a_chok[GA];
  long a_pabs[GA];
  int bp_[GB], b_r[GB], b_s[GB], b_c0[GB];
  int b_n[GB], b_ohw[GB];
  bool b_rscok[GB];
  long b_pabs[GB];
  const bf16* b_lin[GB];
#pragma unroll
  for (int j = 0; j < GA; ++j) {
    const int d = j * TPB + tid;
    wg_decode_chunk(d, a_p[j], a_ch[j]);
    a_chok[j] = kb + a_ch[j] < q.K;
    a_src[j] = q.dy + (p_begin + a_p[j]) * q.K + kb + a_ch[j];
    a_pabs[j] = p_begin + a_p[j];
  }
#pragma unroll
  for (int j = 0; j < GB; ++j) {
    const int d = j * TPB + tid;
    int bch;
    wg_decode_chunk(d, bp_[j], bch);
    const long rsc = rb + bch;
    b_rscok[j] = rsc < q.RSC;
    const long rr = b_rscok[j] ? rsc : 0;
    b_c0[j] = (int)(rr % q.C);
    const int rs = (int)(rr / q.C);
    b_r[j] = rs / q.S;
    b_s[j] = rs - b_r[j] * q.S;
    const long pp = p_begin + bp_[j];
    const int ohw = q.OH * q.OW;
    const long ppc = pp < q.P ? pp : 0;
    b_n[j] = (int)(ppc / ohw);
    const int rem = (int)(ppc - (long)b_n[j] * ohw);
    const int oh0 = rem / q.OW;
    b_ohw[j] = (oh0 << 16) | (rem - oh0 * q.OW);
    b_pabs[j] = pp;
    if (R1) b_lin[j] = q.x + (p_begin + bp_[j]) * q.C + b_c0[j];
  }

  auto stage = [&](int buf, int t) {
    short* la = aimg(buf);
    short* lb = bimg(buf);
    const long plim = p_end;
#pragma unroll
    for (int j = 0; j < GA; ++j) {
      const int d = j * TPB + tid;
      const bf16* src =
          (a_chok[j] && a_pabs[j] + (long)t * WG_BKP < plim)
              ? a_src[j] + (long)t * WG_BKP * q.K
              : q.zero;
      glds16(src, la + d * 8);
    }
#pragma unroll
    for (int j = 0; j < GB; ++j) {
      const int d = j * TPB + tid;
      const bf16* src = q.zero;
      if (R1) {
        if (b_rscok[j] && b_pabs[j] + (long)t * WG_BKP < plim)
          src = b_lin[j] + (long)t * WG_BKP * q.C;
      } else if (b_rscok[j] && b_pabs[j] + (long)t * WG_BKP < plim) {
        const int ih = (b_ohw[j] >> 16) * q.stride + b_r[j] - q.pad;
        const int iw = (b_ohw[j] & 0xffff) * q.stride + b_s[j] - q.pad;
        if (ih >= 0 && ih < q.H && iw >= 0 && iw < q.W)
          src = q.x + (((long)b_n[j] * q.H + ih) * q.W + iw) * q.C +
                b_c0[j];
      }
      glds16(src, lb + d * 8);
      if (!R1) {
        int oh = b_ohw[j] >> 16, ow = (b_ohw[j] & 0xffff) + WG_BKP;
        while (ow >= q.OW) {
          ow -= q.OW;
          if (++oh == q.OH) {
            oh = 0;
            ++b_n[j];
          }
        }
        b_ohw[j] = (oh << 16) | ow;
      }
    }
  };

  const int wk = wid / WC;
  const int wc = wid % WC;
  f32x4 acc[MFS][NFS];
#pragma unroll
  for (int i = 0; i < MFS; ++i)
#pragma unroll
    for (int j = 0; j < NFS; ++j) acc[i][j] = {0.f, 0.f, 0.f, 0.f};

  stage(0, 0);
  if (!RING2 && nsteps > 1) {
    stage(1, 1);
    wait_vmcnt<GA + GB>();
  } else {
    wait_vmcnt<0>();
  }
  __builtin_amdgcn_s_barrier();

  for (int t = 0; t < nsteps; ++t) {
    const short* la = aimg(t % NBUF);
    const short* lb = bimg(t % NBUF);
#pragma unroll
    for (int ks = 0; ks < 2; ++ks) {
      bf16x8 af[MFS], bf_[NFS];
#pragma unroll
      for (int nf = 0; nf < NFS; ++nf)
        bf_[nf] = wg_tr_frag(lb, wc * NFS + nf, ks, lane);
#pragma unroll
      for (int mf = 0; mf < MFS; ++mf)
        af[mf] = wg_tr_frag(la, wk * MFS + mf, ks, lane);
      asm volatile("s_waitcnt lgkmcnt(0)" ::: "memory");
      __builtin_amdgcn_sched_barrier(0);
      __builtin_amdgcn_s_setprio(1);
#pragma unroll
      for (int mf = 0; mf < MFS; ++mf)
#pragma unroll
        for (int nf = 0; nf < NFS; ++nf)
          acc[mf][nf] = __builtin_amdgcn_mfma_f32_16x16x32_bf16(
              af[mf], bf_[nf], acc[mf][nf], 0, 0, 0);
      __builtin_amdgcn_s_setprio(0);
    }
    if (RING2) {
      if (t + 1 < nsteps) stage((t + 1) % 2, t + 1);
      wait_vmcnt<0>();
    } else if (t + 2 < nsteps) {
      stage((t + 2) % 3, t + 2);
      wait_vmcnt<GA + GB>();
    } else {
      wait_vmcnt<0>();
    }
    __builtin_amdgcn_s_barrier();
  }

  float* out = (q.split_p > 1)
                   ? q.part + (long)ps_idx * q.K * q.RSC
                   : q.dw;
#pragma unroll
  for (int mf = 0; mf < MFS; ++mf) {
#pragma unroll
    for (int reg = 0; reg < 4; ++reg) {
      const long k = kb + (wk * MFS + mf) * 16 + (lane >> 4) * 4 + reg;
      if (k >= q.K) continue;
#pragma unroll
      for (int nf = 0; nf < NFS; ++nf) {
        const long rsc = rb + (wc * NFS + nf) * 16 + (lane & 15);
        if (rsc < q.RSC) out[k * q.RSC + rsc] = acc[mf][nf][reg];
      }
    }
  }
}

__global__ void wgrad_combine_kernel(const float* __restrict__ part,
                                     float* __restrict__ dw, long total,
                                     long stride_elems, int split) {
  const int ps0 = blockIdx.y * 64;
  const int ps1 = min(ps0 + 64, split);
  const long i0 = (long)blockIdx.x * blockDim.x + threadIdx.x;
  const long gstride = (long)gridDim.x * blockDim.x;
  for (long i = i0; i < total; i += gstride) {
    float s = 0.f;
    for (int ps = ps0; ps < ps1; ++ps) s += part[ps * stride_elems + i];
    if (gridDim.y > 1)
      atomicAdd(&dw[i], s);
    else
      dw[i] = s;
  }
}

template <int TKt, int TRt, int WR, int WC, int TPB, bool RING2>
void wg_launch(const WgradParams& q, bool r1, unsigned grid, size_t lds,
               hipStream_t stream) {
  if (r1)
    hipLaunchKernelGGL(
        (conv_wgrad2_kernel<TKt, TRt, WR, WC, TPB, true, RING2>),
        dim3(grid), dim3(TPB), lds, stream, q);
  else
    hipLaunchKernelGGL(
        (conv_wgrad2_kernel<TKt, TRt, WR, WC, TPB, false, RING2>),
        dim3(grid), dim3(TPB), lds, stream, q);
}

}

ddlb::ConvWgradPlan ddlb::conv_wgrad_plan(int N, int C, int K, int OH,
                                          int OW, int R, int S, int stride,
                                          int pad, long part_cap) {
  ConvWgradPlan pl;
  const long P = (long)N * OH * OW;
  const long RSC = (long)R * S * C;
  const bool bigK = K >= 128, bigR = RSC >= 128;
  pl.tk = bigK ? 128 : 64;
  pl.tr = bigR ? 128 : 64;
  pl.nk = (K + pl.tk - 1) / pl.tk;
  pl.nr = (RSC + pl.tr - 1) / pl.tr;
  long split = 2048 / i64max(pl.nk * pl.nr, 1);
  split = i64max(i64min(split, (P + WG_BKP - 1) / WG_BKP), 1);
  split = i64min(split, 256);
  if (split > 1)
    split = i64min(split, part_cap / i64max((long)K * RSC, 1));
  split = i64max(split, 1);
  pl.split = split;
  pl.ring = (bigK && bigR) ? 2 : 3;
  pl.r1 = (R == 1 && S == 1 && stride == 1 && pad == 0);
  pl.p_per = (P + split - 1) / split;
  pl.steps = (pl.p_per + WG_BKP - 1) / WG_BKP;
  pl.tail = pl.p_per - (pl.steps - 1) * WG_BKP;
  pl.psb = split > 1 ? (split + 63) / 64 : 0;
  return pl;
}

void ddlb::launch_conv_wgrad(const void* x, const void* dy, float* dw,
                             float* part_ws, long part_cap, const void* zero,
                             int N, int H, int W, int C, int K, int OH, int OW,
                             int R, int S, int stride, int pad,
                             hipStream_t stream) {
  WgradParams q;
  q.x = (const bf16*)x;
  q.dy = (const bf16*)dy;
  q.dw = dw;
  q.part = part_ws;
  q.zero = (const bf16*)zero;
  q.N = N; q.H = H; q.W = W; q.C = C; q.K = K; q.OH = OH; q.OW = OW;
  q.R = R; q.S = S; q.stride = stride; q.pad = pad;
  q.P = (long)N * OH * OW;
  q.RSC = (long)R * S * C;

  const ConvWgradPlan pl = conv_wgrad_plan(N, C, K, OH, OW, R, S, stride,
                                           pad, part_cap);
  q.split_p = (int)pl.split;
  const size_t lds = pl.ring * WG_BKP * (pl.tk + pl.tr) * sizeof(bf16);
  const bool r1 = pl.r1 != 0;
  const unsigned grid = (unsigned)(pl.nk * pl.nr * q.split_p);
  if (pl.tk == 128 && pl.tr == 128)
    wg_launch<128, 128, 2, 4, 512, true>(q, r1, grid, lds, stream);
  else if (pl.tr == 128)
    wg_launch<64, 128, 1, 4, 256, false>(q, r1, grid, lds, stream);
  else if (pl.tk == 128)
    wg_launch<128, 64, 4, 1, 256, false>(q, r1, grid, lds, stream);
  else
    wg_launch<64, 64, 1, 4, 256, false>(q, r1, grid, lds, stream);
  if (q.split_p > 1) {
    const long total = q.K * q.RSC;
    const int blocks = (int)i64min((total + 255) / 256, 2048);
    const int psb = (int)pl.psb;
    if (psb > 1)
      hipMemsetAsync(dw, 0, total * sizeof(float), stream);
    hipLaunchKernelGGL(wgrad_combine_kernel, dim3(blocks, psb),
                       dim3(256), 0,
                       stream, part_ws, dw, total, total, q.split_p);
  }
  HIP_CHECK_LAST();
}
```

ddlbench_amd/ops/csrc/launchers.h:

```cpp
#pragma once

#include <hip/hip_runtime.h>
#include <stdint.h>

namespace ddlb {

template <typename T>
void launch_fused_sgd(uintptr_t* params, uintptr_t* grads, uintptr_t* moms,
                      const int64_t* prefix, int n_tensors, int64_t total,
                      float lr, float momentum, float wd, int first_step,
                      hipStream_t stream);
template <typename T>
void launch_fused_adam(uintptr_t* params, uintptr_t* grads, uintptr_t* ms,
                       uintptr_t* vs, const int64_t* prefix, int n_tensors,
                       int64_t total, float lr, float beta1, float beta2,
                       float eps, float wd, float bc1, float bc2,
                       int decoupled, hipStream_t stream);

void set_bn_variant(int v);
int64_t bn_reduce_gridS(int64_t N, int64_t C, int64_t HW, int nhwc,
                        int elsize);
template <typename T>
void launch_bn_stats(const T*, double*, int64_t, int64_t, int64_t, int64_t,
                     int, hipStream_t);
void launch_bn_finalize(double*, float*, float*, float*, float*,
                        int64_t, int64_t, double, float, float,
                        hipStream_t);
template <typename T>
bool launch_bn_apply(const T*, const T*, T*, const float*, const float*,
                     const float*, const float*, unsigned char*, int64_t,
                     int64_t, int64_t, int, int, hipStream_t);
template <typename T>
void launch_bn_bwd_reduce(const T*, const T*, const T*, const float*,
                          const float*, double*, const unsigned char*,
                          int64_t, int64_t, int64_t, int64_t,
                          int, int, hipStream_t);
void launch_bn_bwd_finalize(double*, const float*, const float*,
                            float*, float*, float*, int64_t, int64_t,
                            double, int, hipStream_t);
template <typename T>
void launch_bn_bwd_dx(const T*, const T*, const T*, const float*,
                      const float*, const float*, T*, T*,
                      const unsigned char*, int64_t, int64_t,
                      int64_t, int, int, hipStream_t);

template <typename T>
void launch_ce_fwd(const T*, const int64_t*, float*, float*, int64_t,
                   int64_t, hipStream_t);
template <typename T>
void launch_ce_bwd(const T*, const int64_t*, const float*, const float*, T*,
                   int64_t, int64_t, hipStream_t);

void launch_conv_igemm(const void* a, const void* b, void* out,
                       const void* zero, int N, int H, int W, int Cin,
                       int K, int OH, int OW, int R, int S, int stride,
                       int pad, int dgrad, const void* add,
                       hipStream_t stream);

struct ConvIgemmLaunch {
  int v2;
  int mode;
  int bm, bn;
  int lin;
  long M, Nd, Kd;
  int cls_a, cls_b, r0, s0, nr, ns, nh, nw;
};
struct ConvIgemmPlan {
  int n;
  ConvIgemmLaunch e[4];
};
ConvIgemmPlan conv_igemm_plan(int N, int H, int W, int Cin, int K, int OH,
                              int OW, int R, int S, int stride, int pad,
                              int dgrad);

constexpr long kConvWgradPartCap = 8L << 20;
struct ConvWgradPlan {
  int tk, tr;
  int ring;
  int r1;
  long nk, nr;
  long split;
  long p_per;
  long steps;
  long tail;
  long psb;
};
ConvWgradPlan conv_wgrad_plan(int N, int C, int K, int OH, int OW, int R,
                              int S, int stride, int pad, long part_cap);
void launch_conv_wgrad(const void* x, const void* dy, float* dw,
                       float* part_ws, long part_cap, const void* zero,
                       int N, int H, int W, int C, int K, int OH, int OW,
                       int R, int S, int stride, int pad,
                       hipStream_t stream);

void launch_conv_stem_fwd(const void* x, const void* w, void* y, int N,
                          int H, int W, int C, int K, int OH, int OW, int R,
                          int stride, int pad, hipStream_t stream);
void launch_conv_stem_wgrad(const void* x, const void* dy, float* dw,
                            float* part, int N, int H, int W, int C, int K,
                            int OH, int OW, int R, int stride, int pad,
                            hipStream_t stream);
int conv_stem_wgrad_chunks(int N, int OH, int OW, int K);

void launch_maxpool_fwd(const void*, void*, unsigned char*, int64_t,
                        int64_t, int, int, int, int, int, int, int,
                        hipStream_t);
void launch_maxpool_bwd(const void*, const unsigned char*, void*,
                        int64_t, int64_t, int, int, int, int, int, int,
                        int, hipStream_t);

template <typename T>
void launch_revert_varlen(const T*, T*, const int64_t*, int64_t, int64_t,
                          int64_t, hipStream_t);
void launch_varlen_mask(const int64_t*, uint8_t*, int64_t, int64_t,
                        hipStream_t);

template <typename T>
void launch_dw3x3_fwd(const T*, const float*, T*, int64_t, int64_t, int64_t,
                      int64_t, int64_t, int64_t, int, int, hipStream_t);
template <typename T>
void launch_dw3x3_bwd_dx(const T*, const float*, T*, int64_t, int64_t,
                         int64_t, int64_t, int64_t, int64_t, int, int,
                         hipStream_t);
template <typename T>
void launch_dw3x3_bwd_dw(const T*, const T*, double*, int64_t, int64_t,
                         int64_t, int64_t, int64_t, int64_t, int, int,
                         hipStream_t);

}
```

setup.py:

```python

import os
import sys
from pathlib import Path

os.environ.setdefault("PYTORCH_ROCM_ARCH", "gfx950")
os.environ.setdefault("MAX_JOBS", str(min(8, os.cpu_count() or 4)))

from setuptools import setup
from torch.utils.cpp_extension import BuildExtension, CUDAExtension

ROOT = Path(__file__).resolve().parent
CSRC = ROOT / "ddlbench_amd" / "ops" / "csrc"

KERNEL_SOURCES = [
    "bindings.hip",
    "bn_act.hip",
    "conv_mfma.hip",
    "conv_mfma2.hip",
    "conv_stem.hip",
    "conv_wgrad.hip",
    "cross_entropy.hip",
    "depthwise_conv.hip",
    "fused_sgd.hip",
    "maxpool.hip",
    "seq_utils.hip",
]
sources = [str(CSRC / s) for s in KERNEL_SOURCES]

setup(
    name="ddlbench_amd_ops",
    version="0.1.0",
    ext_modules=[
        CUDAExtension(
            name="ddlbench_amd.ops._hip_ops",
            sources=sources,
            extra_compile_args={
                "cxx": ["-O3", "-std=c++17"],
                "nvcc": ["-O3", "-std=c++17"],
            },
        )
    ],
    cmdclass={"build_ext": BuildExtension.with_options(use_ninja=True)},
)
```

Before: 8803 images/sec.

## Fuse conv wgrad bf16 output, add native weight transpose, rework BN finalize

Conv weight-grad now writes bf16 in (K,C,R,S) channels-last layout directly from the kernel, or through an ordered split combine, which removes the fp32 output plus the separate permute/cast. A dedicated LDS-tiled transpose kernel builds the dgrad weight layout in place of a PyTorch permute+contiguous. BatchNorm partial sums become fp32 slabs, and finalize becomes a 2-D tiled kernel that combines partials across blocks with atomic tickets. Together these cut small kernel launches and memory traffic in the backward pass, at the cost of more complex synchronization and slightly different accumulation precision.

```diff
diff --git a/ddlbench_amd/ops/conv.py b/ddlbench_amd/ops/conv.py
--- a/ddlbench_amd/ops/conv.py
+++ b/ddlbench_amd/ops/conv.py
@@ -10,6 +10,8 @@
 from ddlbench_amd import ops as _ops
 
 _WGRAD = os.environ.get("DDLB_WGRAD", "mfma")
+
+NATIVE_TAIL = os.environ.get("DDLB_CONV_TAIL", "native") != "eager"
 
 _CL = torch.channels_last
 
@@ -25,12 +27,21 @@
     dy = dy.contiguous(memory_format=_CL)
     dx = dw = None
     if ctx.needs_input_grad[0]:
-        w_perm = weight.permute(1, 2, 3, 0).contiguous()
+        if NATIVE_TAIL and (weight.is_contiguous(memory_format=_CL)
+                            or weight.is_contiguous()):
+            w_perm = ext.conv_weight_dgrad_layout(weight)
+        else:
+            w_perm = weight.permute(1, 2, 3, 0).contiguous()
         dx = ext.conv_igemm_dgrad(dy, w_perm, x.size(0), x.size(1),
                                   x.size(2), x.size(3), ctx.stride,
                                   ctx.pad, add)
     if ctx.needs_input_grad[1]:
-        if _WGRAD == "mfma":
+        if _WGRAD == "mfma" and NATIVE_TAIL \
+                and weight.dtype == torch.bfloat16:
+            dw = ext.conv_igemm_wgrad_bf16(x, dy, weight.shape[2],
+                                           weight.shape[3], ctx.stride,
+                                           ctx.pad)
+        elif _WGRAD == "mfma":
             dw = _dw_to_weight_layout(
                 ext.conv_igemm_wgrad(x, dy, weight.shape[2],
                                      weight.shape[3], ctx.stride,
diff --git a/ddlbench_amd/ops/csrc/bindings.hip b/ddlbench_amd/ops/csrc/bindings.hip
--- a/ddlbench_amd/ops/csrc/bindings.hip
+++ b/ddlbench_amd/ops/csrc/bindings.hip
@@ -60,10 +60,22 @@
   return cached_ws(zp, like, at::kBFloat16, 16, 0, true);
 }
 
-torch::Tensor bn_sums_workspace(const torch::Tensor& like, int64_t C,
-                                int64_t S) {
-  static WsCache ws;
-  return cached_ws(ws, like, at::kDouble, 2 * C * S, 1 << 18);
+struct BnWorkspace {
+  BnWorkspacePlan plan;
+  torch::Tensor sums, part, tickets;
+};
+BnWorkspace bn_workspace(const torch::Tensor& x, int64_t N, int64_t C,
+                         int64_t HW, bool nhwc) {
+  static WsCache ws_sums, ws_part, ws_tickets;
+  BnWorkspace w;
+  w.plan = bn_workspace_plan(N, C, HW, nhwc, (int)x.element_size());
+  w.sums = cached_ws(ws_sums, x, at::kDouble, (w.plan.slab_bytes + 7) / 8,
+                     1 << 18);
+  w.part = cached_ws(ws_part, x, at::kDouble,
+                     std::max<int64_t>(w.plan.part_doubles, 1), 1 << 16);
+  w.tickets = cached_ws(ws_tickets, x, at::kInt, w.plan.cchunks, 1 << 10,
+                        true);
+  return w;
 }
 
 void check_conv_operand(const torch::Tensor& t, const char* name,
@@ -152,16 +164,16 @@
   torch::Tensor mean = torch::empty({C}, fopt);
   torch::Tensor invstd = torch::empty({C}, fopt);
   if (training) {
-    const int64_t S =
-        bn_reduce_gridS(N, C, HW, nhwc, (int)x.element_size());
-    torch::Tensor sums = bn_sums_workspace(x, C, S);
+    const BnWorkspace ws = bn_workspace(x, N, C, HW, nhwc);
+    const int64_t S = ws.plan.S;
     dispatch_f32_bf16(x, [&](auto tag) {
       using T = decltype(tag);
-      launch_bn_stats<T>(dptr<T>(x), dptr<double>(sums), N, C, HW, S, nhwc,
+      launch_bn_stats<T>(dptr<T>(x), ws.sums.data_ptr(), N, C, HW, S, nhwc,
                          s);
     });
     launch_bn_finalize(
-        dptr<double>(sums), dptr<float>(mean), dptr<float>(invstd),
+        ws.sums.data_ptr(), ws.plan.slab_f32, dptr<double>(ws.part),
+        dptr<unsigned>(ws.tickets), dptr<float>(mean), dptr<float>(invstd),
         running_mean ? dptr<float>(*running_mean) : nullptr,
         running_var ? dptr<float>(*running_var) : nullptr, C, S,
         (double)(N * HW), (float)eps, (float)momentum, s);
@@ -205,8 +217,8 @@
   const int64_t N = x.size(0), C = x.size(1), HW = x.size(2) * x.size(3);
   auto s = cur_stream();
   auto fopt = x.options().dtype(at::kFloat);
-  const int64_t S = bn_reduce_gridS(N, C, HW, nhwc, (int)x.element_size());
-  torch::Tensor sums = bn_sums_workspace(x, C, S);
+  const BnWorkspace ws = bn_workspace(x, N, C, HW, nhwc);
+  const int64_t S = ws.plan.S;
   torch::Tensor dgamma = torch::empty({C}, fopt);
   torch::Tensor dbeta = torch::empty({C}, fopt);
   torch::Tensor k = torch::empty({3, C}, fopt);
@@ -224,9 +236,11 @@
     using T = decltype(tag);
     const T* yp = y_opt ? dptr<T>(*y_opt) : nullptr;
     launch_bn_bwd_reduce<T>(dptr<T>(dy), yp, dptr<T>(x), dptr<float>(mean),
-                            dptr<float>(invstd), dptr<double>(sums), mp, N,
+                            dptr<float>(invstd), ws.sums.data_ptr(), mp, N,
                             C, HW, S, (int)act, nhwc, s);
-    launch_bn_bwd_finalize(dptr<double>(sums), dptr<float>(gamma),
+    launch_bn_bwd_finalize(ws.sums.data_ptr(), ws.plan.slab_f32,
+                           dptr<double>(ws.part), dptr<unsigned>(ws.tickets),
+                           dptr<float>(gamma),
                            dptr<float>(invstd), dptr<float>(dgamma),
                            dptr<float>(dbeta), dptr<float>(k), C, S,
                            (double)(N * HW), training, s);
@@ -330,9 +344,10 @@
   return dx;
 }
 
-torch::Tensor conv_igemm_wgrad(torch::Tensor x, torch::Tensor dy,
-                               int64_t R, int64_t S, int64_t stride,
-                               int64_t pad) {
+static torch::Tensor conv_wgrad_impl(const torch::Tensor& x,
+                                     const torch::Tensor& dy, int64_t R,
+                                     int64_t S, int64_t stride, int64_t pad,
+                                     bool out_bf16) {
   TORCH_CHECK(x.dim() == 4 && dy.dim() == 4, "conv_wgrad: 4-D tensors only");
   check_conv_operand(x, "x", "conv_wgrad");
   check_conv_operand(dy, "dy", "conv_wgrad");
@@ -345,15 +360,56 @@
   TORCH_CHECK(K >= 1, "conv_wgrad: empty dy");
   check_conv_geometry("conv_wgrad", N, H, W, R, S, stride, pad);
   check_conv_dy("conv_wgrad", dy, N, H, W, R, S, stride, pad);
-  auto dw = torch::empty({K, R * S * C},
-                         x.options().dtype(at::kFloat));
+  auto dw = out_bf16
+                ? torch::empty({K, R, S, C}, x.options()).permute({0, 3, 1, 2})
+                : torch::empty({K, R * S * C}, x.options().dtype(at::kFloat));
   static WsCache wgws;
   auto part = cached_ws(wgws, x, at::kFloat, kConvWgradPartCap);
-  launch_conv_wgrad(x.data_ptr(), dy.data_ptr(), dw.data_ptr<float>(),
+  launch_conv_wgrad(x.data_ptr(), dy.data_ptr(),
+                    out_bf16 ? nullptr : dw.data_ptr<float>(),
                     part.data_ptr<float>(), (long)part.numel(),
                     zero_page(x).data_ptr(), N, H, W, C, K, OH, OW, (int)R,
-                    (int)S, (int)stride, (int)pad, cur_stream());
+                    (int)S, (int)stride, (int)pad, cur_stream(),
+                    out_bf16 ? dw.data_ptr() : nullptr);
   return dw;
+}
+
+torch::Tensor conv_igemm_wgrad(torch::Tensor x, torch::Tensor dy,
+                               int64_t R, int64_t S, int64_t stride,
+                               int64_t pad) {
+  return conv_wgrad_impl(x, dy, R, S, stride, pad, false);
+}
+
+torch::Tensor conv_igemm_wgrad_bf16(torch::Tensor x, torch::Tensor dy,
+                                    int64_t R, int64_t S, int64_t stride,
+                                    int64_t pad) {
+  return conv_wgrad_impl(x, dy, R, S, stride, pad, true);
+}
+
+torch::Tensor conv_weight_dgrad_layout(torch::Tensor weight) {
+  TORCH_CHECK(weight.is_cuda() && weight.scalar_type() == at::kBFloat16,
+              "conv_weight_dgrad_layout: bf16 HIP tensors only");
+  TORCH_CHECK(weight.dim() == 4,
+              "conv_weight_dgrad_layout: weight must be 4-D (K,C,R,S)");
+  const int64_t K = weight.size(0), C = weight.size(1);
+  const int64_t R = weight.size(2), S = weight.size(3);
+  TORCH_CHECK(K >= 8 && C >= 8 && K % 8 == 0 && C % 8 == 0 && R >= 1 &&
+                  S >= 1,
+              "conv_weight_dgrad_layout needs K % 8 == 0 and C % 8 == 0");
+  const bool cl = weight.is_contiguous(at::MemoryFormat::ChannelsLast);
+  TORCH_CHECK(cl || weight.is_contiguous(),
+              "conv_weight_dgrad_layout: weight must be channels_last or "
+              "contiguous");
+  auto out = torch::empty({C, R, S, K}, weight.options().memory_format(
+                                            at::MemoryFormat::Contiguous));
+  const int64_t RS = R * S;
+  if (cl)
+    launch_weight_transpose(weight.data_ptr(), out.data_ptr(), RS, K, C,
+                            RS * C, C, RS * K, K, cur_stream());
+  else
+    launch_weight_transpose(weight.data_ptr(), out.data_ptr(), 1, K, C * RS,
+                            C * RS, 0, K, 0, cur_stream());
+  return out;
 }
 
 py::list conv_igemm_plan_py(int64_t N, int64_t C, int64_t H, int64_t W,
@@ -587,6 +643,13 @@
         py::arg("add") = py::none());
   m.def("conv_igemm_wgrad", &conv_igemm_wgrad,
         "NHWC bf16 MFMA implicit-GEMM conv weight-grad (fp32 out)");
+  m.def("conv_igemm_wgrad_bf16", &conv_igemm_wgrad_bf16,
+        "MFMA weight-grad straight to bf16 (K,C,R,S) channels_last",
+        py::arg("x"), py::arg("dy"), py::arg("R"), py::arg("S"),
+        py::arg("stride"), py::arg("pad"));
+  m.def("conv_weight_dgrad_layout", &conv_weight_dgrad_layout,
+        "bf16 weight (K,C,R,S) -> contiguous (C,R,S,K) for the dgrad kernels",
+        py::arg("weight"));
   m.def("conv_igemm_plan", &conv_igemm_plan_py,
         "launches conv_igemm_fwd/dgrad make for a shape (host only)",
         py::arg("N"), py::arg("C"), py::arg("H"), py::arg("W"),
diff --git a/ddlbench_amd/ops/csrc/bn_act.hip b/ddlbench_amd/ops/csrc/bn_act.hip
--- a/ddlbench_amd/ops/csrc/bn_act.hip
+++ b/ddlbench_amd/ops/csrc/bn_act.hip
@@ -97,7 +97,7 @@
 
 template <typename T>
 __global__ void bn_stats_nhwc_vec_kernel(const T* __restrict__ x,
-                                         double* __restrict__ sums,
+                                         float* __restrict__ sums,
                                          int64_t rows, int64_t C, int CG8) {
   typedef __attribute__((ext_vector_type(8))) short short8x;
   __shared__ float tmp[2][256][8];
@@ -141,8 +141,8 @@
       }
 #pragma unroll
     for (int j = 0; j < 8; ++j) {
-      sums[((int64_t)blockIdx.y * 2 + 0) * C + c0 + j] = (double)s[j];
-      sums[((int64_t)blockIdx.y * 2 + 1) * C + c0 + j] = (double)ss[j];
+      sums[((int64_t)blockIdx.y * 2 + 0) * C + c0 + j] = s[j];
+      sums[((int64_t)blockIdx.y * 2 + 1) * C + c0 + j] = ss[j];
     }
   }
 }
@@ -194,34 +194,131 @@
   }
 }
 
-__global__ void bn_finalize_kernel(const double* __restrict__ sums,
-                                   float* __restrict__ mean,
-                                   float* __restrict__ invstd,
-                                   float* __restrict__ running_mean,
-                                   float* __restrict__ running_var,
-                                   int64_t C, int64_t S, double count,
-                                   float eps, float momentum) {
-  __shared__ double tmp[16];
-  const int64_t c = blockIdx.x;
-  double s = 0.0, ss = 0.0;
-  for (int64_t b = threadIdx.x; b < S; b += blockDim.x) {
-    s += sums[(b * 2 + 0) * C + c];
-    ss += sums[(b * 2 + 1) * C + c];
-  }
-  auto op = [](double v) { return wave_reduce_sum(v); };
-  s = block_reduce(s, tmp, op, 0.0);
+#define BN_FIN_CH 32
+#define BN_FIN_TY 8
+#define BN_FIN_ROWS 32
+#define BN_FIN_YMAX 64
+
+struct BnFinParams {
+  const void* sums;
+  double* part;
+  unsigned* tickets;
+  int64_t C, S;
+  int rows_per;
+  double count;
+  float* mean; float* invstd; float* running_mean; float* running_var;
+  float eps, momentum;
+  const float* gamma; const float* invstd_in;
+  float* dgamma; float* dbeta; float* k;
+  int training;
+};
+
+template <typename ST, bool BWD>
+__global__ __launch_bounds__(BN_FIN_CH * BN_FIN_TY)
+void bn_finalize_kernel(BnFinParams q) {
+  __shared__ double sh[2][BN_FIN_TY][BN_FIN_CH];
+  __shared__ int is_last;
+  const int tx = threadIdx.x, ty = threadIdx.y;
+  const int t = ty * BN_FIN_CH + tx;
+  const int Y = gridDim.y;
+  const int64_t c = (int64_t)blockIdx.x * BN_FIN_CH + tx;
+  const ST* sums = static_cast<const ST*>(q.sums);
+
+  double a0 = 0.0, a1 = 0.0;
+  if (c < q.C) {
+    const int64_t r0 = (int64_t)blockIdx.y * q.rows_per;
+    const int64_t r1 = i64min(r0 + q.rows_per, q.S);
+    int64_t r = r0 + ty;
+    for (; r + 3 * BN_FIN_TY < r1; r += 4 * BN_FIN_TY) {
+      ST v0[4], v1[4];
+#pragma unroll
+      for (int j = 0; j < 4; ++j) {
+        v0[j] = sums[((r + j * BN_FIN_TY) * 2 + 0) * q.C + c];
+        v1[j] = sums[((r + j * BN_FIN_TY) * 2 + 1) * q.C + c];
+      }
+#pragma unroll
+      for (int j = 0; j < 4; ++j) {
+        a0 += (double)v0[j];
+        a1 += (double)v1[j];
+      }
+    }
+    for (; r < r1; r += BN_FIN_TY) {
+      a0 += (double)sums[(r * 2 + 0) * q.C + c];
+      a1 += (double)sums[(r * 2 + 1) * q.C + c];
+    }
+  }
+  sh[0][ty][tx] = a0;
+  sh[1][ty][tx] = a1;
   __syncthreads();
-  ss = block_reduce(ss, tmp, op, 0.0);
-  if (threadIdx.x != 0) return;
-  const double m = s / count;
-  double var = ss / count - m * m;
-  var = var < 0.0 ? 0.0 : var;
-  mean[c] = (float)m;
-  invstd[c] = (float)rsqrt(var + (double)eps);
-  if (running_mean != nullptr) {
-    const double unbiased = count > 1.0 ? var * count / (count - 1.0) : var;
-    running_mean[c] = (1.f - momentum) * running_mean[c] + momentum * (float)m;
-    running_var[c] = (1.f - momentum) * running_var[c] + momentum * (float)unbiased;
+  double v = 0.0;
+  if (t < 2 * BN_FIN_CH) {
+#pragma unroll
+    for (int j = 0; j < BN_FIN_TY; ++j) v += sh[ty][j][tx];
+  }
+
+  if (Y > 1) {
+    double* part = q.part + (int64_t)blockIdx.x * Y * 2 * BN_FIN_CH;
+    if (t < 2 * BN_FIN_CH) part[(int64_t)blockIdx.y * 2 * BN_FIN_CH + t] = v;
+    asm volatile("s_waitcnt vmcnt(0)" ::: "memory");
+    __syncthreads();
+    if (t == 0) {
+      __builtin_amdgcn_fence(__ATOMIC_RELEASE, "agent");
+      asm volatile("s_waitcnt vmcnt(0)" ::: "memory");
+      const unsigned ticket = __hip_atomic_fetch_add(
+          &q.tickets[blockIdx.x], 1u, __ATOMIC_RELAXED,
+          __HIP_MEMORY_SCOPE_AGENT);
+      const int last = ticket == (unsigned)(Y - 1);
+      if (last) {
+        __builtin_amdgcn_fence(__ATOMIC_ACQUIRE, "agent");
+        asm volatile("s_waitcnt vmcnt(0)" ::: "memory");
+        __hip_atomic_store(&q.tickets[blockIdx.x], 0u, __ATOMIC_RELAXED,
+                           __HIP_MEMORY_SCOPE_AGENT);
+      }
+      is_last = last;
+    }
+    __syncthreads();
+    if (!is_last) return;
+    a0 = 0.0;
+    a1 = 0.0;
+    for (int y = ty; y < Y; y += BN_FIN_TY) {
+      a0 += part[(int64_t)(y * 2 + 0) * BN_FIN_CH + tx];
+      a1 += part[(int64_t)(y * 2 + 1) * BN_FIN_CH + tx];
+    }
+    sh[0][ty][tx] = a0;
+    sh[1][ty][tx] = a1;
+    __syncthreads();
+    v = 0.0;
+    if (t < 2 * BN_FIN_CH) {
+#pragma unroll
+      for (int j = 0; j < BN_FIN_TY; ++j) v += sh[ty][j][tx];
+    }
+  }
+
+  __syncthreads();
+  if (t < 2 * BN_FIN_CH) sh[ty][0][tx] = v;
+  __syncthreads();
+  if (t >= BN_FIN_CH || c >= q.C) return;
+  const double s0 = sh[0][0][tx], s1 = sh[1][0][tx];
+  if (!BWD) {
+    const double m = s0 / q.count;
+    double var = s1 / q.count - m * m;
+    var = var < 0.0 ? 0.0 : var;
+    q.mean[c] = (float)m;
+    q.invstd[c] = (float)rsqrt(var + (double)q.eps);
+    if (q.running_mean != nullptr) {
+      const double unbiased =
+          q.count > 1.0 ? var * q.count / (q.count - 1.0) : var;
+      q.running_mean[c] = (1.f - q.momentum) * q.running_mean[c] +
+                          q.momentum * (float)m;
+      q.running_var[c] = (1.f - q.momentum) * q.running_var[c] +
+                         q.momentum * (float)unbiased;
+    }
+  } else {
+    q.dgamma[c] = (float)s1;
+    q.dbeta[c] = (float)s0;
+    q.k[c] = q.gamma[c] * q.invstd_in[c];
+    q.k[q.C + c] = q.training ? (float)(s0 / q.count) : 0.f;
+    q.k[2 * q.C + c] = q.training ? (float)(s1 / q.count) : 0.f;
   }
 }
 
@@ -574,7 +671,7 @@
 __global__ void bn_bwd_reduce_nhwc_vec_kernel(
     const T* __restrict__ dy, const T* __restrict__ y,
     const T* __restrict__ x, const float* __restrict__ mean,
-    const float* __restrict__ invstd, double* __restrict__ sums,
+    const float* __restrict__ invstd, float* __restrict__ sums,
     const unsigned char* __restrict__ msk,
     int64_t rows, int64_t C, int CG8) {
   typedef __attribute__((ext_vector_type(8))) short short8x;
@@ -645,37 +742,10 @@
       }
 #pragma unroll
     for (int j = 0; j < 8; ++j) {
-      sums[((int64_t)blockIdx.y * 2 + 0) * C + c0 + j] = (double)sdy[j];
-      sums[((int64_t)blockIdx.y * 2 + 1) * C + c0 + j] = (double)sdyx[j];
-    }
-  }
-}
-
-__global__ void bn_bwd_finalize_kernel(const double* __restrict__ sums,
-                                       const float* __restrict__ gamma,
-                                       const float* __restrict__ invstd,
-                                       float* __restrict__ dgamma,
-                                       float* __restrict__ dbeta,
-                                       float* __restrict__ k,
-                                       int64_t C, int64_t S, double count,
-                                       int training) {
-  __shared__ double tmp[16];
-  const int64_t c = blockIdx.x;
-  double sdy = 0.0, sdyx = 0.0;
-  for (int64_t b = threadIdx.x; b < S; b += blockDim.x) {
-    sdy += sums[(b * 2 + 0) * C + c];
-    sdyx += sums[(b * 2 + 1) * C + c];
-  }
-  auto op = [](double v) { return wave_reduce_sum(v); };
-  sdy = block_reduce(sdy, tmp, op, 0.0);
-  __syncthreads();
-  sdyx = block_reduce(sdyx, tmp, op, 0.0);
-  if (threadIdx.x != 0) return;
-  dgamma[c] = (float)sdyx;
-  dbeta[c] = (float)sdy;
-  k[c] = gamma[c] * invstd[c];
-  k[C + c] = training ? (float)(sdy / count) : 0.f;
-  k[2 * C + c] = training ? (float)(sdyx / count) : 0.f;
+      sums[((int64_t)blockIdx.y * 2 + 0) * C + c0 + j] = sdy[j];
+      sums[((int64_t)blockIdx.y * 2 + 1) * C + c0 + j] = sdyx[j];
+    }
+  }
 }
 
 template <typename T, int ACT, bool ADD>
@@ -731,8 +801,46 @@
   return i64max(S, 1);
 }
 
+static bool bn_slab_f32(int64_t rows, int64_t C, int nhwc, int elsize) {
+  return nhwc && elsize == 2 && bn_reduce_geom(rows, C, elsize).vec;
+}
+
+static int64_t bn_fin_Y(int64_t S) {
+  return i64min((S + BN_FIN_ROWS - 1) / BN_FIN_ROWS, BN_FIN_YMAX);
+}
+
+ddlb::BnWorkspacePlan ddlb::bn_workspace_plan(int64_t N, int64_t C,
+                                              int64_t HW, int nhwc,
+                                              int elsize) {
+  BnWorkspacePlan p;
+  p.S = bn_reduce_gridS(N, C, HW, nhwc, elsize);
+  p.slab_f32 = bn_slab_f32(N * HW, C, nhwc, elsize) ? 1 : 0;
+  p.slab_bytes = p.S * 2 * C * (p.slab_f32 ? 4 : 8);
+  p.cchunks = (C + BN_FIN_CH - 1) / BN_FIN_CH;
+  p.Y = bn_fin_Y(p.S);
+  p.part_doubles = p.Y > 1 ? p.cchunks * p.Y * 2 * BN_FIN_CH : 0;
+  return p;
+}
+
+template <bool BWD>
+static void bn_finalize_launch(BnFinParams q, bool slab_f32,
+                               hipStream_t stream) {
+  const int64_t Y = bn_fin_Y(q.S);
+  q.rows_per = (int)((q.S + Y - 1) / Y);
+  const dim3 grid((unsigned)((q.C + BN_FIN_CH - 1) / BN_FIN_CH),
+                  (unsigned)Y);
+  const dim3 block(BN_FIN_CH, BN_FIN_TY);
+  if (slab_f32)
+    hipLaunchKernelGGL((bn_finalize_kernel<float, BWD>), grid, block, 0,
+                       stream, q);
+  else
+    hipLaunchKernelGGL((bn_finalize_kernel<double, BWD>), grid, block, 0,
+                       stream, q);
+  HIP_CHECK_LAST();
+}
+
 template <typename T>
-void ddlb::launch_bn_stats(const T* x, double* sums, int64_t N, int64_t C,
+void ddlb::launch_bn_stats(const T* x, void* sums, int64_t N, int64_t C,
                            int64_t HW, int64_t S, int nhwc,
                            hipStream_t stream) {
   const int block = 256;
@@ -743,33 +851,38 @@
       const int CG8 = (int)i64min(C / 8, 64);
       hipLaunchKernelGGL((bn_stats_nhwc_vec_kernel<T>),
                          dim3(g.cblocks, S),
-                         dim3(block), 0, stream, x, sums, rows, C, CG8);
+                         dim3(block), 0, stream, x, (float*)sums, rows, C,
+                         CG8);
     } else if (g.vec && sizeof(T) == 4) {
       const int CG4 = (int)i64min(C / 4, 64);
       hipLaunchKernelGGL(bn_stats_nhwc_vec_f32_kernel, dim3(g.cblocks, S),
-                         dim3(block), 0, stream, (const float*)x, sums,
-                         rows, C, CG4);
+                         dim3(block), 0, stream, (const float*)x,
+                         (double*)sums, rows, C, CG4);
     } else {
       const int CG = C >= 64 ? 64 : (int)C;
       hipLaunchKernelGGL((bn_stats_nhwc_kernel<T>), dim3(g.cblocks, S),
-                         dim3(block), 0, stream, x, sums, rows, C, CG);
+                         dim3(block), 0, stream, x, (double*)sums, rows, C,
+                         CG);
     }
   } else {
     hipLaunchKernelGGL((bn_stats_kernel<T>), dim3(C, S), dim3(block), 0,
-                       stream, x, sums, N, C, HW);
+                       stream, x, (double*)sums, N, C, HW);
   }
   HIP_CHECK_LAST();
 }
 
-void ddlb::launch_bn_finalize(double* sums, float* mean, float* invstd,
+void ddlb::launch_bn_finalize(const void* sums, int slab_f32, double* part,
+                              unsigned* tickets, float* mean, float* invstd,
                               float* rm, float* rv, int64_t C, int64_t S,
                               double count, float eps, float momentum,
                               hipStream_t stream) {
-  const int block = 1024;
-  hipLaunchKernelGGL(bn_finalize_kernel, dim3((unsigned)C),
-                     dim3(block), 0, stream, sums, mean, invstd, rm, rv, C,
-                     S, count, eps, momentum);
-  HIP_CHECK_LAST();
+  BnFinParams q = {};
+  q.sums = sums; q.part = part; q.tickets = tickets;
+  q.C = C; q.S = S; q.count = count;
+  q.mean = mean; q.invstd = invstd;
+  q.running_mean = rm; q.running_var = rv;
+  q.eps = eps; q.momentum = momentum;
+  bn_finalize_launch<false>(q, slab_f32 != 0, stream);
 }
 
 template <typename T>
@@ -843,7 +956,7 @@
 template <typename T>
 void ddlb::launch_bn_bwd_reduce(const T* dy, const T* y, const T* x,
                                 const float* mean, const float* invstd,
-                                double* sums, const unsigned char* msk,
+                                void* sums_v, const unsigned char* msk,
                                 int64_t N, int64_t C, int64_t HW, int64_t S,
                                 int act, int nhwc, hipStream_t stream) {
   const int block = 256;
@@ -856,7 +969,8 @@
 #define CASE(ACT, MSK)                                                      \
       hipLaunchKernelGGL((bn_bwd_reduce_nhwc_vec_kernel<T, ACT, MSK>),      \
                          dim3(g.cblocks, S), dim3(block), 0, stream, dy,    \
-                         y, x, mean, invstd, sums, msk, rows, C, CG8)
+                         y, x, mean, invstd, (float*)sums_v, msk, rows, C,  \
+                         CG8)
       if (act == 0) CASE(0, false);
       else if (act == 1) { if (masked) CASE(1, true); else CASE(1, false); }
       else { if (masked) CASE(2, true); else CASE(2, false); }
@@ -866,7 +980,8 @@
 #define CASE(ACT, MSK)                                                      \
       hipLaunchKernelGGL((bn_bwd_reduce_nhwc_kernel<T, ACT, MSK>),          \
                          dim3(g.cblocks, S), dim3(block), 0, stream, dy,    \
-                         y, x, mean, invstd, sums, msk, rows, C, CG)
+                         y, x, mean, invstd, (double*)sums_v, msk, rows, C, \
+                         CG)
       if (act == 0) CASE(0, false);
       else if (act == 1) { if (masked) CASE(1, true); else CASE(1, false); }
       else { if (masked) CASE(2, true); else CASE(2, false); }
@@ -876,7 +991,7 @@
 #define CASE(ACT)                                                          \
     hipLaunchKernelGGL((bn_bwd_reduce_kernel<T, ACT>), dim3(C, S),         \
                        dim3(block), 0, stream, dy, y, x, mean, invstd,     \
-                       sums, N, C, HW)
+                       (double*)sums_v, N, C, HW)
     if (act == 0) CASE(0);
     else if (act == 1) CASE(1);
     else CASE(2);
@@ -885,16 +1000,19 @@
   HIP_CHECK_LAST();
 }
 
-void ddlb::launch_bn_bwd_finalize(double* sums, const float* gamma,
-                                  const float* invstd, float* dgamma,
-                                  float* dbeta, float* k, int64_t C, int64_t S,
-                                  double count, int training,
-                                  hipStream_t stream) {
-  const int block = 1024;
-  hipLaunchKernelGGL(bn_bwd_finalize_kernel, dim3((unsigned)C),
-                     dim3(block), 0, stream, sums, gamma, invstd, dgamma,
-                     dbeta, k, C, S, count, training);
-  HIP_CHECK_LAST();
+void ddlb::launch_bn_bwd_finalize(const void* sums, int slab_f32,
+                                  double* part, unsigned* tickets,
+                                  const float* gamma, const float* invstd,
+                                  float* dgamma, float* dbeta, float* k,
+                                  int64_t C, int64_t S, double count,
+                                  int training, hipStream_t stream) {
+  BnFinParams q = {};
+  q.sums = sums; q.part = part; q.tickets = tickets;
+  q.C = C; q.S = S; q.count = count;
+  q.gamma = gamma; q.invstd_in = invstd;
+  q.dgamma = dgamma; q.dbeta = dbeta; q.k = k;
+  q.training = training;
+  bn_finalize_launch<true>(q, slab_f32 != 0, stream);
 }
 
 template <typename T>
@@ -974,14 +1092,14 @@
 
 #define INSTANTIATE(T)                                                        \
   template void ddlb::launch_bn_stats<T>(                                     \
-      const T*, double*, int64_t, int64_t, int64_t, int64_t, int,             \
+      const T*, void*, int64_t, int64_t, int64_t, int64_t, int,             \
       hipStream_t);                                                           \
   template bool ddlb::launch_bn_apply<T>(                                     \
       const T*, const T*, T*, const float*, const float*, const float*,       \
       const float*, unsigned char*, int64_t, int64_t, int64_t, int, int,      \
       hipStream_t);                                                           \
   template void ddlb::launch_bn_bwd_reduce<T>(                                \
-      const T*, const T*, const T*, const float*, const float*, double*,      \
+      const T*, const T*, const T*, const float*, const float*, void*,        \
       const unsigned char*, int64_t, int64_t, int64_t, int64_t, int, int,     \
       hipStream_t);                                                           \
   template void ddlb::launch_bn_bwd_dx<T>(                                    \
diff --git a/ddlbench_amd/ops/csrc/conv_weight_layout.hip b/ddlbench_amd/ops/csrc/conv_weight_layout.hip
--- /dev/null
+++ b/ddlbench_amd/ops/csrc/conv_weight_layout.hip
@@ -0,0 +1,72 @@
+
+#include "common.h"
+#include "launchers.h"
+#include <stdint.h>
+#include <stdexcept>
+#include <string>
+
+namespace {
+
+#define WL_TILE 64
+#define WL_PITCH 66
+
+typedef __attribute__((ext_vector_type(8))) unsigned short ushort8x;
+typedef __attribute__((ext_vector_type(4))) unsigned uint4x;
+
+__global__ __launch_bounds__(256)
+void weight_transpose_kernel(const unsigned short* __restrict__ in,
+                             unsigned short* __restrict__ out, long M,
+                             long Nn, long in_rs, long in_bs, long out_rs,
+                             long out_bs) {
+  __shared__ __attribute__((aligned(16)))
+      unsigned short tile[WL_TILE * WL_PITCH];
+  const int t = threadIdx.x;
+  const long n0 = (long)blockIdx.x * WL_TILE;
+  const long m0 = (long)blockIdx.y * WL_TILE;
+  in += (long)blockIdx.z * in_bs;
+  out += (long)blockIdx.z * out_bs;
+#pragma unroll
+  for (int i = 0; i < 2; ++i) {
+    const int m = (t >> 3) + 32 * i;
+    const int n = (t & 7) * 8;
+    if (m0 + m < M && n0 + n < Nn) {
+      const ushort8x v = *reinterpret_cast<const ushort8x*>(
+          in + (m0 + m) * in_rs + n0 + n);
+#pragma unroll
+      for (int j = 0; j < 8; ++j) tile[(n + j) * WL_PITCH + m] = v[j];
+    }
+  }
+  __syncthreads();
+#pragma unroll
+  for (int i = 0; i < 2; ++i) {
+    const int n = (t >> 3) + 32 * i;
+    const int m = (t & 7) * 8;
+    if (n0 + n < Nn && m0 + m < M) {
+      const unsigned* src =
+          reinterpret_cast<const unsigned*>(tile + n * WL_PITCH + m);
+      uint4x v;
+#pragma unroll
+      for (int j = 0; j < 4; ++j) v[j] = src[j];
+      *reinterpret_cast<uint4x*>(out + (n0 + n) * out_rs + m0 + m) = v;
+    }
+  }
+}
+
+}
+
+void ddlb::launch_weight_transpose(const void* in, void* out, long B, long M,
+                                   long Nn, long in_rs, long in_bs,
+                                   long out_rs, long out_bs,
+                                   hipStream_t stream) {
+  if (M % 8 || Nn % 8 || in_rs % 8 || in_bs % 8 || out_rs % 8 || out_bs % 8)
+    throw std::runtime_error(
+        "weight_transpose: dims and strides must be multiples of 8");
+  if (B < 1 || B > 65535 || (M + WL_TILE - 1) / WL_TILE > 65535)
+    throw std::runtime_error("weight_transpose: grid out of range");
+  const dim3 grid((unsigned)((Nn + WL_TILE - 1) / WL_TILE),
+                  (unsigned)((M + WL_TILE - 1) / WL_TILE), (unsigned)B);
+  hipLaunchKernelGGL(weight_transpose_kernel, grid, dim3(256), 0, stream,
+                     (const unsigned short*)in, (unsigned short*)out, M, Nn,
+                     in_rs, in_bs, out_rs, out_bs);
+  HIP_CHECK_LAST();
+}
diff --git a/ddlbench_amd/ops/csrc/conv_wgrad.hip b/ddlbench_amd/ops/csrc/conv_wgrad.hip
--- a/ddlbench_amd/ops/csrc/conv_wgrad.hip
+++ b/ddlbench_amd/ops/csrc/conv_wgrad.hip
@@ -14,6 +14,7 @@
   const bf16* x;
   const bf16* dy;
   float* dw;
+  bf16* dwb;
   float* part;
   const bf16* zero;
   int N, H, W, C, K, OH, OW, R, S, stride, pad;
@@ -226,10 +227,56 @@
 #pragma unroll
       for (int nf = 0; nf < NFS; ++nf) {
         const long rsc = rb + (wc * NFS + nf) * 16 + (lane & 15);
-        if (rsc < q.RSC) out[k * q.RSC + rsc] = acc[mf][nf][reg];
+        if (rsc >= q.RSC) continue;
+        if (q.split_p == 1 && q.dwb != nullptr)
+          q.dwb[k * q.RSC + rsc] = __float2bfloat16(acc[mf][nf][reg]);
+        else
+          out[k * q.RSC + rsc] = acc[mf][nf][reg];
       }
     }
   }
+}
+
+template <typename OutT, int V, int TX, int TY>
+__global__ void wgrad_combine_ordered_kernel(const float* __restrict__ part,
+                                             OutT* __restrict__ dw,
+                                             long total, long stride_elems,
+                                             int split) {
+  __shared__ float sh[TY][TX][V];
+  const int tx = threadIdx.x, ty = threadIdx.y;
+  const long i = ((long)blockIdx.x * TX + tx) * V;
+  const int ps0 = ty * 64;
+  const int ps1 = min(ps0 + 64, split);
+  float s[V];
+#pragma unroll
+  for (int j = 0; j < V; ++j) s[j] = 0.f;
+  if (i < total) {
+#pragma unroll 4
+    for (int ps = ps0; ps < ps1; ++ps) {
+      const float* src = part + ps * stride_elems + i;
+      if constexpr (V == 4) {
+        typedef __attribute__((ext_vector_type(4))) float float4x;
+        const float4x v = *reinterpret_cast<const float4x*>(src);
+#pragma unroll
+        for (int j = 0; j < 4; ++j) s[j] += v[j];
+      } else {
+#pragma unroll
+        for (int j = 0; j < V; ++j) s[j] += src[j];
+      }
+    }
+  }
+  if (TY > 1 && blockDim.y > 1) {
+#pragma unroll
+    for (int j = 0; j < V; ++j) sh[ty][tx][j] = s[j];
+    __syncthreads();
+    if (ty != 0) return;
+    for (int g = 1; g < (int)blockDim.y; ++g)
+#pragma unroll
+      for (int j = 0; j < V; ++j) s[j] += sh[g][tx][j];
+  }
+  if (i >= total) return;
+#pragma unroll
+  for (int j = 0; j < V; ++j) dw[i + j] = from_f32<OutT>(s[j]);
 }
 
 __global__ void wgrad_combine_kernel(const float* __restrict__ part,
@@ -295,11 +342,12 @@
                              float* part_ws, long part_cap, const void* zero,
                              int N, int H, int W, int C, int K, int OH, int OW,
                              int R, int S, int stride, int pad,
-                             hipStream_t stream) {
+                             hipStream_t stream, void* dw_bf16) {
   WgradParams q;
   q.x = (const bf16*)x;
   q.dy = (const bf16*)dy;
   q.dw = dw;
+  q.dwb = (bf16*)dw_bf16;
   q.part = part_ws;
   q.zero = (const bf16*)zero;
   q.N = N; q.H = H; q.W = W; q.C = C; q.K = K; q.OH = OH; q.OW = OW;
@@ -321,7 +369,22 @@
     wg_launch<128, 64, 4, 1, 256, false>(q, r1, grid, lds, stream);
   else
     wg_launch<64, 64, 1, 4, 256, false>(q, r1, grid, lds, stream);
-  if (q.split_p > 1) {
+  if (q.split_p > 1 && q.dwb != nullptr) {
+    const long total = q.K * q.RSC;
+    if (pl.psb > 4)
+      throw std::runtime_error("conv_wgrad: ordered combine needs split <= 256");
+    if (pl.psb <= 1) {
+      const unsigned blocks = (unsigned)((total / 4 + 255) / 256);
+      hipLaunchKernelGGL((wgrad_combine_ordered_kernel<bf16, 4, 256, 1>),
+                         dim3(blocks), dim3(256, 1), 0, stream, part_ws,
+                         q.dwb, total, total, q.split_p);
+    } else {
+      const unsigned blocks = (unsigned)((total + 31) / 32);
+      hipLaunchKernelGGL((wgrad_combine_ordered_kernel<bf16, 1, 32, 4>),
+                         dim3(blocks), dim3(32, (unsigned)pl.psb), 0, stream,
+                         part_ws, q.dwb, total, total, q.split_p);
+    }
+  } else if (q.split_p > 1) {
     const long total = q.K * q.RSC;
     const int blocks = (int)i64min((total + 255) / 256, 2048);
     const int psb = (int)pl.psb;
diff --git a/ddlbench_amd/ops/csrc/launchers.h b/ddlbench_amd/ops/csrc/launchers.h
--- a/ddlbench_amd/ops/csrc/launchers.h
+++ b/ddlbench_amd/ops/csrc/launchers.h
@@ -20,10 +20,20 @@
 void set_bn_variant(int v);
 int64_t bn_reduce_gridS(int64_t N, int64_t C, int64_t HW, int nhwc,
                         int elsize);
+struct BnWorkspacePlan {
+  int64_t S;
+  int slab_f32;
+  int64_t slab_bytes;
+  int64_t cchunks, Y;
+  int64_t part_doubles;
+};
+BnWorkspacePlan bn_workspace_plan(int64_t N, int64_t C, int64_t HW, int nhwc,
+                                  int elsize);
 template <typename T>
-void launch_bn_stats(const T*, double*, int64_t, int64_t, int64_t, int64_t,
-                     int, hipStream_t);
-void launch_bn_finalize(double*, float*, float*, float*, float*,
+void launch_bn_stats(const T*, void* sums, int64_t, int64_t, int64_t,
+                     int64_t, int, hipStream_t);
+void launch_bn_finalize(const void* sums, int slab_f32, double* part,
+                        unsigned* tickets, float*, float*, float*, float*,
                         int64_t, int64_t, double, float, float,
                         hipStream_t);
 template <typename T>
@@ -32,10 +42,11 @@
                      int64_t, int64_t, int, int, hipStream_t);
 template <typename T>
 void launch_bn_bwd_reduce(const T*, const T*, const T*, const float*,
-                          const float*, double*, const unsigned char*,
+                          const float*, void* sums, const unsigned char*,
                           int64_t, int64_t, int64_t, int64_t,
                           int, int, hipStream_t);
-void launch_bn_bwd_finalize(double*, const float*, const float*,
+void launch_bn_bwd_finalize(const void* sums, int slab_f32, double* part,
+                            unsigned* tickets, const float*, const float*,
                             float*, float*, float*, int64_t, int64_t,
                             double, int, hipStream_t);
 template <typename T>
@@ -91,7 +102,11 @@
                        float* part_ws, long part_cap, const void* zero,
                        int N, int H, int W, int C, int K, int OH, int OW,
                        int R, int S, int stride, int pad,
-                       hipStream_t stream);
+                       hipStream_t stream, void* dw_bf16 = nullptr);
+
+void launch_weight_transpose(const void* in, void* out, long B, long M,
+                             long Nn, long in_rs, long in_bs, long out_rs,
+                             long out_bs, hipStream_t stream);
 
 void launch_conv_stem_fwd(const void* x, const void* w, void* y, int N,
                           int H, int W, int C, int K, int OH, int OW, int R,
diff --git a/setup.py b/setup.py
--- a/setup.py
+++ b/setup.py
@@ -18,6 +18,7 @@
     "conv_mfma.hip",
     "conv_mfma2.hip",
     "conv_stem.hip",
+    "conv_weight_layout.hip",
     "conv_wgrad.hip",
     "cross_entropy.hip",
     "depthwise_conv.hip",
```

Result: faster. 9091 images/sec (median of 6 runs) (+3.3%).
